# RishabhSri14/Human-Body-Reconstruction

Measured on NVIDIA B200. Metric: train_rays_per_sec, higher is better.
Workload: dtype bf16 MLP operands (f32 accumulate) / f32 encoder+compositor

## Files before the change

### human_body_reconstruction_b200/_lib.py

```python
from __future__ import annotations

import ctypes as C
import os
import subprocess
import sys
import threading

import torch

_HERE = os.path.dirname(os.path.abspath(__file__))
ROOT = os.path.dirname(_HERE)
CSRC = os.path.join(_HERE, "csrc")
SO_PATH = os.path.join(_HERE, "libhbr_b200.so")
INCLUDE = os.path.join(ROOT, "include")

NVCC_FLAGS = [
    "-gencode", "arch=compute_100a,code=sm_100a", "-O3", "-lineinfo", "-std=c++17",
    "--fmad=true",
    "-Xcompiler", "-fPIC", "-Xcompiler", "-O3", "-Xptxas", "-v",
]

HBR_MAX_LEVELS = 32
HBR_MAX_PEERS, HBR_PEER_MAX_CTAS, HBR_PEER_HANDLE_BYTES = 8, 128, 64
HBR_PEER_FLAG_BYTES = HBR_PEER_MAX_CTAS * HBR_MAX_PEERS * 4
# ... 20 lines not shown

def _deps():
    return [os.path.join(CSRC, f) for f in os.listdir(CSRC) if os.path.isfile(os.path.join(CSRC, f))] + \
        [os.path.join(INCLUDE, "hbr.h")]


def _stale() -> bool:
    if not os.path.exists(SO_PATH):
        return True
    t = os.path.getmtime(SO_PATH)
    return any(os.path.getmtime(d) > t for d in _deps())


def build(force: bool = False, verbose: bool = False) -> str:
    if not force and not _stale():
        return SO_PATH
    bdir = os.path.join(_HERE, "build")
    os.makedirs(bdir, exist_ok=True)
    import fcntl
    with open(os.path.join(bdir, ".lock"), "w") as lockf:
        fcntl.flock(lockf, fcntl.LOCK_EX)
        try:
            if not force and not _stale():
                return SO_PATH
            return _build_locked(bdir, force, verbose)
        finally:
            fcntl.flock(lockf, fcntl.LOCK_UN)


def _build_locked(bdir: str, force: bool, verbose: bool) -> str:
    nvcc = os.environ.get("NVCC", "/usr/local/cuda/bin/nvcc")
    objs, procs = [], []
    for src in sources():
        obj = os.path.join(bdir, os.path.basename(src)[:-3] + ".o")
        objs.append(obj)
        if (not force) and os.path.exists(obj) and os.path.getmtime(obj) > max(os.path.getmtime(d) for d in _deps()):
            continue
        cmd = [nvcc, *NVCC_FLAGS, *os.environ.get("HBR_EXTRA_NVCC", "").split(), "-I", INCLUDE, "-c", src, "-o", obj]
        procs.append((src, subprocess.Popen(cmd, stdout=subprocess.PIPE, stderr=subprocess.STDOUT, text=True)))
    log = []
    for src, p in procs:
        out, _ = p.communicate()
        log.append(f"== {os.path.basename(src)}\n{out}")
        if p.returncode != 0:
            raise RuntimeError(f"nvcc failed for {src}:\n{out}")
    with open(os.path.join(bdir, "ptxas.log"), "a" if not force else "w") as f:
        f.write("\n".join(log))
    if verbose:
        print("\n".join(log))
    tmp_so = os.path.join(bdir, f"libhbr_b200.{os.getpid()}.so.tmp")
    cmd = [nvcc, "-shared", "-o", tmp_so, *objs, "-lcudart"]
    r = subprocess.run(cmd, stdout=subprocess.PIPE, stderr=subprocess.STDOUT, text=True)
    if r.returncode != 0:
        raise RuntimeError(f"link failed:\n{r.stdout}")
    os.replace(tmp_so, SO_PATH)
    return SO_PATH


def build_debug(force: bool = False) -> str:
    dbg = os.path.join(CSRC, "debug")
    srcs = sorted(os.path.join(dbg, f) for f in os.listdir(dbg) if f.endswith(".cu")) + [os.path.join(CSRC, "abi.cu")]
    deps = _deps() + [os.path.join(dbg, f) for f in os.listdir(dbg)]
    if not force and os.path.exists(DEBUG_SO_PATH) and os.path.getmtime(DEBUG_SO_PATH) > max(os.path.getmtime(d) for d in deps):
        return DEBUG_SO_PATH
    nvcc = os.environ.get("NVCC", "/usr/local/cuda/bin/nvcc")
    cmd = [nvcc, *[f for f in NVCC_FLAGS if f not in ("-Xptxas", "-v")], "-I", INCLUDE, "-shared", "-o", DEBUG_SO_PATH, *srcs,
           "-lcudart"]
    r = subprocess.run(cmd, stdout=subprocess.PIPE, stderr=subprocess.STDOUT, text=True)
    if r.returncode != 0:
        raise RuntimeError(f"nvcc failed for the debug library:\n{r.stdout}")
    return DEBUG_SO_PATH


_lib = None
_debug_lib = None
_lock = threading.Lock()

_i64, _i32, _f32, _vp = C.c_int64, C.c_int, C.c_float, C.c_void_p
_geom_p, _dims_p = C.POINTER(HashGeom), C.POINTER(MlpDims)

SIGNATURES = {
    "hbr_abi_version": ([], C.c_int),
    "hbr_last_error": ([], C.c_char_p),
    "hbr_mlp_param_count": ([_dims_p], _i64),
    "hbr_mlp_act_floats": ([], _i64),
    "hbr_hash_encode_fwd": ([_vp, _i32, _i64, _vp, _geom_p, _vp, _i64, _vp], C.c_int),
    "hbr_hash_encode_bwd": ([_vp, _i32, _i64, _vp, _i64, _geom_p, _vp, _i32, _i32, _vp], C.c_int),
    "hbr_hash_encode_dx": ([_vp, _i32, _i64, _vp, _geom_p, _vp, _i64, _vp, _vp], C.c_int),
    "hbr_hash_indices": ([_vp, _i32, _i64, _geom_p, _vp, _vp, _vp], C.c_int),
    "hbr_dir_encode": ([_vp, _i32, _i64, _i32, _i32, _vp, _vp], C.c_int),
    "hbr_mlp_fwd_f32": ([_vp, _i64, _vp, _i64, _i64, _vp, _dims_p, _vp, _vp, _vp], C.c_int),
    "hbr_mlp_bwd_f32": ([_vp, _i64, _vp, _i64, _i64, _vp, _dims_p, _vp, _vp, _vp, _vp, _i64, _vp, _vp, _vp], C.c_int),
    "hbr_mlp_tc_scratch_bytes": ([_dims_p], _i64),
    "hbr_mlp_fwd_tc": ([_vp, _i32, _i64, _vp, _i64, _i64, _vp, _dims_p, _i32, _vp, _vp, _i32, _vp, _vp, _vp], C.c_int),
    "hbr_mlp_bwd_tc": ([_vp, _i32, _i64, _vp, _i64, _i64, _vp, _dims_p, _i32, _vp, _vp, _vp, _i64, _vp, _vp, _f32, _vp, _i32, _i32,
                        _vp, _vp, _vp], C.c_int),
    "hbr_occupancy_update": ([_vp, _i64, _vp, _i64, _vp, _i32, C.POINTER(C.c_float), _f32, _vp, _vp], C.c_int),
    "hbr_compact_samples": ([_vp, _vp, _vp, _i64, _i64, _i64, _vp, _i32, C.POINTER(C.c_float), _f32, _vp, _vp, _vp, _vp, _vp],
                            C.c_int),
    "hbr_hash_encode_fwd_pts": ([_vp, _i64, _vp, _vp, _geom_p, _vp, _i64, _i32, _vp], C.c_int),
    "hbr_hash_encode_bwd_pts": ([_vp, _i64, _vp, _vp, _i64, _geom_p, _vp, _i32, _i32, _vp], C.c_int),
    "hbr_mlp_tc_prepare": ([_vp, _dims_p, _i32, _vp, _vp], C.c_int),
    "hbr_mlp_tc_reduce_grads": ([_dims_p, _i64, _vp, _vp, _vp], C.c_int),
    "hbr_strat_depths": ([_vp, _vp, _f32, _f32, _i64, _vp, _vp], C.c_int),
    "hbr_mse_pair_fwd": ([_vp, _vp, _vp, _i64, _f32, _vp, _vp], C.c_int),
    "hbr_mse_pair_bwd": ([_vp, _vp, _vp, _i64, _f32, _vp, _vp, _vp, _vp], C.c_int),
    "hbr_hash_encode_fwd_rays": ([_vp, _vp, _vp, _i64, _i64, _i64, _vp, _geom_p, _vp, _i64, _i32, _vp], C.c_int),
    "hbr_field_bwd_rays_tc": ([_vp, _vp, _vp, _vp, _i64, _i64, _i64, _geom_p, _vp, _vp, _dims_p, _i32, _vp, _vp, _vp, _vp, _vp, _f32,
                               _vp, _i32, _i32, _vp], C.c_int),
    "hbr_field_fwd_rays_tc": ([_vp, _vp, _vp, _i64, _i64, _i64, _vp, _geom_p, _vp, _vp, _dims_p, _i32, _vp, _vp, _vp, _i32, _vp],
                              C.c_int),
    "hbr_hash_encode_bwd_rays": ([_vp, _vp, _vp, _i64, _i64, _i64, _vp, _i64, _geom_p, _vp, _i32, _i32, _vp], C.c_int),
    "hbr_field_fwd_tc": ([_vp, _i64, _vp, _geom_p, _vp, _i64, _vp, _dims_p, _i32, _vp, _vp, _vp, _vp], C.c_int),
    "hbr_field_bwd_tc": ([_vp, _i64, _geom_p, _vp, _i64, _vp, _dims_p, _i32, _vp, _vp, _vp, _vp, _vp, _vp, _f32, _vp, _vp],
                         C.c_int),
    "hbr_adam_step": ([_vp, _vp, _vp, _vp, _i64, C.c_double, C.c_double, C.c_double, C.c_double, C.c_double, _i32, _i64,
                       C.c_double, _vp, _vp], C.c_int),
    "hbr_adam_tick": ([_vp, _vp, _vp], C.c_int),
    "hbr_adam_step_dev": ([_vp, _vp, _vp, _vp, _i64, _vp, C.c_double, C.c_double, C.c_double, C.c_double, _i32, _vp, C.c_double,
                           _vp, _vp, _vp], C.c_int),
    "hbr_ray_gen": ([_vp, _i64, _i32, _i32, _f32, _f32, _f32, _f32, _vp, _i64, _i64, _vp, _i32, _vp, _vp, _vp, _vp, _vp, _vp],
                    C.c_int),
    "hbr_ray_bbox": ([_vp, _i64, _i32, _i32, _f32, _f32, _f32, _f32, _f32, _f32, _vp, _vp], C.c_int),
    "hbr_peer_alloc": ([C.POINTER(_vp), _i64], C.c_int),
    "hbr_peer_free": ([_vp], C.c_int),
    "hbr_peer_export": ([_vp, C.POINTER(C.c_ubyte)], C.c_int),
    "hbr_peer_import": ([C.POINTER(C.c_ubyte), C.POINTER(_vp)], C.c_int),
    "hbr_peer_release": ([_vp], C.c_int),
    "hbr_allreduce_peer": ([C.POINTER(_vp), C.POINTER(_vp), _vp, _i32, _i32, _i64, _f32, _i32, _vp, _vp], C.c_int),
    "hbr_hash_bwd_stream_tiles": ([_i64], _i64),
    "hbr_hash_encode_bwd_stream": ([_vp, _i32, _i64, _vp, _i64, _geom_p, _vp, C.POINTER(C.c_int), _i32, _vp, _vp], C.c_int),
    "hbr_hash_encode_bwd_rays_stream": ([_vp, _vp, _vp, _i64, _i64, _i64, _vp, _i64, _geom_p, _vp, C.POINTER(C.c_int), _i32, _vp,
                                         _vp], C.c_int),
    "hbr_hash_bwd_lm_ctas": ([_i64], _i64),
    "hbr_hash_encode_bwd_lm": ([_vp, _i32, _i64, _vp, _geom_p, _vp, C.POINTER(C.c_int), _i32, _vp, _vp], C.c_int),
    "hbr_hash_encode_bwd_rays_lm": ([_vp, _vp, _vp, _i64, _i64, _i64, _vp, _geom_p, _vp, C.POINTER(C.c_int), _i32, _vp, _vp],
                                    C.c_int),
    "hbr_allreduce_peer_stream": ([C.POINTER(_vp), C.POINTER(_vp), _vp, _i32, _i32, _i32, C.POINTER(_i64), C.POINTER(_i64),
                                   C.POINTER(C.c_uint), C.POINTER(C.c_int), _vp, _f32, _i32, _vp, _vp], C.c_int),
    "hbr_ray_points": ([_vp, _vp, _vp, _i64, _i64, _i64, _vp, _vp], C.c_int),
    "hbr_occupancy_mask": ([_vp, _i64, _vp, _i32, C.POINTER(C.c_float), _f32, _vp, _vp], C.c_int),
    "hbr_composite_fwd": ([_vp, _i64, _vp, _i64, _vp, _i64, _vp, _f32, _vp, _vp, _i64, _i64, _vp, _vp, _f32, _vp], C.c_int),
    "hbr_composite_bwd": ([_vp, _i64, _vp, _i64, _vp, _i64, _vp, _f32, _vp, _vp, _i64, _i64, _vp, _vp, _i64, _vp, _i64, _f32, _vp],
                          C.c_int),
    "hbr_composite_maps_fwd": ([_vp, _i64, _vp, _i64, _vp, _i64, _vp, _f32, _vp, _vp, _i64, _i64, _vp, _vp, _vp, _vp, _f32, _vp],
                               C.c_int),
    "hbr_composite_maps_bwd": ([_vp, _i64, _vp, _i64, _vp, _i64, _vp, _f32, _vp, _vp, _i64, _i64, _vp, _vp, _vp, _vp, _i64, _vp,
                                _i64, _f32, _vp], C.c_int),
    "hbr_hier_sample": ([_vp, _vp, _vp, _vp, _i64, _i64, _i32, _vp, _vp], C.c_int),
    "hbr_composite_sdf_fwd": ([_vp, _i64, _vp, _i64, _i32, _vp, _i64, _i64, _vp, _vp, _vp], C.c_int),
    "hbr_composite_sdf_bwd": ([_vp, _i64, _vp, _i64, _i32, _vp, _i64, _i64, _vp, _vp, _vp, _i64, _vp, _i64, _vp, _vp], C.c_int),
    "hbr_sdf_stencil_points": ([_vp, _i64, _f32, C.POINTER(C.c_float), C.POINTER(C.c_float), _vp, _vp], C.c_int),
    "hbr_sdf_eikonal_fwd": ([_vp, _i64, _f32, _vp, _vp, _vp], C.c_int),
    "hbr_sdf_eikonal_bwd": ([_vp, _i64, _f32, _vp, _vp, _vp], C.c_int),
    "hbr_grid_points": ([C.POINTER(C.c_double), C.POINTER(C.c_double), _i32, _i64, _i64, _vp, _vp], C.c_int),
    "hbr_grid_density": ([C.POINTER(C.c_double), C.POINTER(C.c_double), _i32, _i64, _i64, _vp, _geom_p, _vp, _dims_p,
                          _vp, _vp, _vp, _vp, _i64, _i32, _vp], C.c_int),
    "hbr_mlp_density_tf32x3": ([_vp, _i64, _vp, _dims_p, _vp, _vp], C.c_int),
    "hbr_mc_count": ([_vp, _i32, _i32, _i32, _f32, _i32, _i32, _vp, _vp], C.c_int),
    "hbr_mc_emit": ([_vp, _i32, _i32, _i32, _f32, _i32, _i32, _vp, _vp, _i64, _vp, _i64, _vp, _vp], C.c_int),
    "hbr_grid_interp": ([_vp, _i32, _i32, _i32, _i32, _vp, _i64, _vp, _vp], C.c_int),
}

DEBUG_SIGNATURES = {
    "hbr_debug_umma": ([_i32, _i32, _vp, _vp, _vp, _i32, _i32, _vp], C.c_int),
    "hbr_debug_umma_bench": ([_i32, _i32, _i32, _i32, _i32, _vp, _vp], C.c_int),
# ... 134 lines not shown
```

### human_body_reconstruction_b200/csrc/abi.cu

```cuda
#include "common.cuh"
#include <string.h>

namespace hbr {

char* err_buf() {
  static thread_local char buf[512] = {0};
  return buf;
}

int fail(int code, const char* fmt, ...) {
  va_list ap;
  va_start(ap, fmt);
  vsnprintf(err_buf(), 512, fmt, ap);
  va_end(ap);
  return code;
}

int sm_count() {
  static thread_local int cached_dev = -1, cached = 0;
  int dev = 0;
  if (cudaGetDevice(&dev) != cudaSuccess) return 148;
  if (dev != cached_dev) {
    cudaDeviceProp p;
    if (cudaGetDeviceProperties(&p, dev) != cudaSuccess) return 148;
    cached = p.multiProcessorCount;
    cached_dev = dev;
  }
  return cached;
}

}

extern "C" int hbr_abi_version(void) { return HBR_ABI_VERSION; }
extern "C" const char* hbr_last_error(void) { return hbr::err_buf(); }
```

### human_body_reconstruction_b200/csrc/common.cuh

```cuda
#pragma once
#include <cuda_runtime.h>
#include <cuda_fp16.h>
#include <cuda_bf16.h>
#include <stdint.h>
#include <stdio.h>
#include <stdarg.h>
#include "../../include/hbr.h"

namespace hbr {

char* err_buf();
int fail(int code, const char* fmt, ...);

#define HBR_REQUIRE(cond, ...)                                  \
  do {                                                          \
    if (!(cond)) return ::hbr::fail(HBR_ERR_ARG, __VA_ARGS__);  \
  } while (0)

#define HBR_CUDA(expr)                                                                         \
  do {                                                                                         \
    cudaError_t e__ = (expr);                                                                  \
    if (e__ != cudaSuccess)                                                                    \
      return ::hbr::fail(HBR_ERR_CUDA, "%s failed: %s (%s:%d)", #expr, cudaGetErrorString(e__), \
                         __FILE__, __LINE__);                                                  \
  } while (0)

#define HBR_LAUNCH_CHECK() HBR_CUDA(cudaGetLastError())

static inline cudaStream_t as_stream(void* s) { return reinterpret_cast<cudaStream_t>(s); }
static inline int64_t ceil_div(int64_t a, int64_t b) { return (a + b - 1) / b; }
static inline int64_t min64(int64_t a, int64_t b) { return a < b ? a : b; }
int sm_count();

constexpr uint32_t kPrimeY = 2654435761u;
constexpr uint32_t kPrimeZ = 805459861u;
constexpr long long kPrimeY64 = -1640531535LL;
constexpr long long kPrimeZ64 = 805459861LL;

struct HashGeom {
  float mu[3];
  float sigma;
  int L, F, E;
  uint32_t T;
  float scale[HBR_MAX_LEVELS];
};

static inline HashGeom to_device_geom(const hbr_hash_geom& g) {
  HashGeom d;
  for (int i = 0; i < 3; ++i) d.mu[i] = g.mu[i];
  d.sigma = g.sigma;
  d.L = g.L; d.F = g.F; d.E = g.E; d.T = g.T;
  for (int i = 0; i < HBR_MAX_LEVELS; ++i) d.scale[i] = i < g.L ? g.scale[i] : 0.f;
  return d;
}

static inline bool is_pow2(uint32_t v) { return v && !(v & (v - 1)); }

template <typename XT> __device__ __forceinline__ float load_coord(const XT* p);
template <> __device__ __forceinline__ float load_coord<float>(const float* p) { return __ldg(p); }
template <> __device__ __forceinline__ float load_coord<__half>(const __half* p) { return __half2float(__ldg(p)); }

__device__ __forceinline__ void cell_of(float x, float mu, float sigma, float scale, long long& cell, float& frac) {
  const float u = __fmul_rn(__fdiv_rn(__fsub_rn(x, mu), sigma), scale);
  cell = __float2ll_rz(u);
  frac = __fsub_rn(u, __ll2float_rn(cell));
}

template <bool POW2>
__device__ __forceinline__ uint32_t hash_corner(long long cx, long long cy, long long cz, uint32_t T) {
  if (POW2) {
    const uint32_t h = (uint32_t)cx ^ ((uint32_t)cy * kPrimeY) ^ ((uint32_t)cz * kPrimeZ);
    return h & (T - 1);
  } else {
    const unsigned long long a = (unsigned long long)cx;
    const unsigned long long b = (unsigned long long)cy * (unsigned long long)kPrimeY64;
    const unsigned long long c = (unsigned long long)cz * (unsigned long long)kPrimeZ64;
    long long v = (long long)(a ^ b ^ c);
    long long r = v % (long long)T;
    if (r < 0) r += (long long)T;
    return (uint32_t)r;
  }
}

__device__ __forceinline__ void corner_weights(float fx, float fy, float fz, float w[8]) {
  const float wx[2] = {__fsub_rn(1.f, fx), fx};
  const float wy[2] = {__fsub_rn(1.f, fy), fy};
  const float wz[2] = {__fsub_rn(1.f, fz), fz};
#pragma unroll
  for (int c = 0; c < 8; ++c) w[c] = __fmul_rn(__fmul_rn(wx[c & 1], wy[(c >> 1) & 1]), wz[(c >> 2) & 1]);
}

template <bool POW2>
__device__ __forceinline__ void corner_indices(long long ix, long long iy, long long iz, uint32_t T, uint32_t idx[8]) {
  if (POW2) {
    const uint32_t a[2] = {(uint32_t)ix, (uint32_t)ix + 1u};
    const uint32_t b0 = (uint32_t)iy * kPrimeY, c0 = (uint32_t)iz * kPrimeZ;
    const uint32_t b[2] = {b0, b0 + kPrimeY};
    const uint32_t c[2] = {c0, c0 + kPrimeZ};
#pragma unroll
    for (int k = 0; k < 8; ++k) idx[k] = (a[k & 1] ^ b[(k >> 1) & 1] ^ c[(k >> 2) & 1]) & (T - 1);
  } else {
#pragma unroll
    for (int k = 0; k < 8; ++k) idx[k] = hash_corner<false>(ix + (k & 1), iy + ((k >> 1) & 1), iz + ((k >> 2) & 1), T);
  }
}

constexpr unsigned kFull = 0xffffffffu;

__device__ __forceinline__ float warp_sum(float v) {
#pragma unroll
  for (int o = 16; o > 0; o >>= 1) v += __shfl_xor_sync(kFull, v, o);
  return v;
}
__device__ __forceinline__ float warp_incl_scan(float v, int lane) {
#pragma unroll
// ... 17 lines not shown
```

### human_body_reconstruction_b200/csrc/composite.cu

```cuda
#include "common.cuh"
#include <math_constants.h>

namespace hbr {

constexpr int kRaysPerCta = 8;

__global__ void ray_points_kernel(const float* __restrict__ o, const float* __restrict__ d, const float* __restrict__ t,
                                  long long t_rs, long long R, long long S, float* __restrict__ pts) {
  const long long i = (long long)blockIdx.x * blockDim.x + threadIdx.x;
  if (i >= R * S) return;
  const long long r = i / S, s = i - r * S;
  const float tt = __ldg(t + r * t_rs + s);
#pragma unroll
  for (int k = 0; k < 3; ++k) pts[i * 3 + k] = __fadd_rn(__ldg(o + r * 3 + k), __fmul_rn(__ldg(d + r * 3 + k), tt));
}

struct Mu3 { float v[3]; };
__global__ void occupancy_kernel(const float* __restrict__ pts, long long n, const uint8_t* __restrict__ grid, int G,
                                 Mu3 mu, float sigma, uint8_t* __restrict__ mask) {
  const long long i = (long long)blockIdx.x * blockDim.x + threadIdx.x;
  if (i >= n) return;
  long long q[3];
#pragma unroll
  for (int k = 0; k < 3; ++k) {
    const float u = __fmul_rn(__fdiv_rn(__fsub_rn(__ldg(pts + i * 3 + k), mu.v[k]), sigma), (float)G);
    long long c = __float2ll_rz(u);
    if (c < 0) c += G;
    c = c < 0 ? 0 : (c >= G ? G - 1 : c);
    q[k] = c;
  }
  mask[i] = grid[(q[0] * G + q[1]) * G + q[2]] ? 1 : 0;
}

template <typename XT>
__global__ void dir_encode_kernel(const XT* __restrict__ d, long long n, int dim, int nf, float* __restrict__ out) {
  const long long i = (long long)blockIdx.x * blockDim.x + threadIdx.x;
  const long long total = n * dim * nf;
  if (i >= total) return;
  const int k = (int)(i % nf);
  const long long rc = i / nf;
  float s, c;
  if (sizeof(XT) == 2) {
    const float x = __half2float(reinterpret_cast<const __half*>(d)[rc]);
    const float two_x = __half2float(__float2half_rn(2.f * x));
    const float a = __half2float(__float2half_rn(two_x * (float)k));
    s = __half2float(__float2half_rn(sinf(a)));
    c = __half2float(__float2half_rn(cosf(a)));
  } else {
    const float x = reinterpret_cast<const float*>(d)[rc];
    const float a = __fmul_rn(__fmul_rn(2.f, x), (float)k);
    s = sinf(a);
    c = cosf(a);
  }
  float* o = out + rc * (2 * nf);
  o[k] = s;
  o[nf + k] = c;
}

struct SampleIn {
  float delta, sig, p;
  bool keep;
};

__device__ __forceinline__ long long sample_row(const int32_t* __restrict__ rowmap, long long gs, int s, int S) {
  return rowmap == nullptr ? gs : (s < S ? (long long)__ldg(rowmap + gs) : -1);
}

__device__ __forceinline__ SampleIn load_sample(const float* __restrict__ tr, const float* __restrict__ sigma,
                                                long long sig_st, const uint8_t* __restrict__ mask, long long gs,
                                                int s, int S, float dnr, bool& live, long long row) {
  SampleIn q;
  live = s < S && row >= 0 && (mask == nullptr || mask[gs]);
  float delta = 0.f;
  if (s + 1 < S) delta = __fsub_rn(__ldg(tr + s + 1), __ldg(tr + s));
  q.delta = __fmul_rn(delta, dnr);
  const float raw = live ? __ldg(sigma + row * sig_st) : 0.f;
  q.keep = !(raw < -10.f);
  q.sig = q.keep ? raw : -10.f;
  q.p = s < S ? __fmul_rn(q.sig, q.delta) : 0.f;
  return q;
}

template <bool MAPS>
__global__ void __launch_bounds__(kRaysPerCta * 32)
composite_fwd_kernel(const float* __restrict__ t, long long t_rs, const float* __restrict__ rgb, long long rgb_st,
                     const float* __restrict__ sigma, long long sig_st, const float* __restrict__ dn, float dn_scalar,
                     const uint8_t* __restrict__ mask, const int32_t* __restrict__ rowmap, long long R, int S,
                     float* __restrict__ C, float* __restrict__ w_out, float ert_tau, float* __restrict__ depth,
                     float* __restrict__ opac) {
  const int lane = threadIdx.x & 31;
  const long long ray = (long long)blockIdx.x * kRaysPerCta + (threadIdx.x >> 5);
  if (ray >= R) return;
  const float* tr = t + ray * t_rs;
  const float dnr = dn ? __ldg(dn + ray) : dn_scalar;
  float carry = 0.f, c0 = 0.f, c1 = 0.f, c2 = 0.f, dsum = 0.f, asum = 0.f;
  for (int s0 = 0; s0 < S; s0 += 32) {
    const int s = s0 + lane;
    const long long gs = ray * S + s;
    bool live;
    const long long row = sample_row(rowmap, gs, s, S);
    const SampleIn q = load_sample(tr, sigma, sig_st, mask, gs, s, S, dnr, live, row);
    const float incl = carry + warp_incl_scan(q.p, lane);
    float prev = __shfl_up_sync(kFull, incl, 1);
    if (lane == 0) prev = carry;
    const float T = s == 0 ? 1.f : expf(-prev);
    const float alpha = 1.f - expf(-q.p);
    const float w = s < S ? __fmul_rn(T, alpha) : 0.f;
    if (s < S) {
      if (w_out) w_out[gs] = w;
      if (MAPS) {
        dsum += w * __ldg(tr + s);
        asum += w;
      }
      if (live) {
        const float* c = rgb + row * rgb_st;
        c0 += w * __ldg(c + 0);
        c1 += w * __ldg(c + 1);
        c2 += w * __ldg(c + 2);
      }
    }
    carry = __shfl_sync(kFull, incl, 31);
    if (carry > ert_tau) {
      if (w_out)
        for (int s2 = s0 + 32 + lane; s2 < S; s2 += 32) w_out[ray * S + s2] = 0.f;
      break;
    }
  }
  c0 = warp_sum(c0); c1 = warp_sum(c1); c2 = warp_sum(c2);
  if (lane == 0) { C[ray * 3 + 0] = c0; C[ray * 3 + 1] = c1; C[ray * 3 + 2] = c2; }
  if (MAPS) {
    dsum = warp_sum(dsum); asum = warp_sum(asum);
    if (lane == 0) {
      if (depth) depth[ray] = dsum;
      if (opac) opac[ray] = asum;
    }
  }
}

template <int NCH, bool MAPS>
__global__ void __launch_bounds__(kRaysPerCta * 32)
composite_bwd_kernel(const float* __restrict__ t, long long t_rs, const float* __restrict__ rgb, long long rgb_st,
                     const float* __restrict__ sigma, long long sig_st, const float* __restrict__ dn, float dn_scalar,
                     const uint8_t* __restrict__ mask, const int32_t* __restrict__ rowmap, long long R, int S,
                     const float* __restrict__ gC, float* __restrict__ drgb, long long drgb_st, float* __restrict__ dsig,
                     long long dsig_st, float ert_tau, const float* __restrict__ gD, const float* __restrict__ gA) {
  const int lane = threadIdx.x & 31;
  const long long ray = (long long)blockIdx.x * kRaysPerCta + (threadIdx.x >> 5);
  if (ray >= R) return;
  const float* tr = t + ray * t_rs;
  const float dnr = dn ? __ldg(dn + ray) : dn_scalar;
  float g0 = 0.f, g1 = 0.f, g2 = 0.f, gd = 0.f, ga = 0.f;
  if (!MAPS || gC) { g0 = __ldg(gC + ray * 3 + 0); g1 = __ldg(gC + ray * 3 + 1); g2 = __ldg(gC + ray * 3 + 2); }
  if (MAPS) {
    if (gD) gd = __ldg(gD + ray);
    if (gA) ga = __ldg(gA + ray);
  }
  const bool packed = drgb_st == 4 && dsig_st == 4 && dsig == drgb + 3;

  float Tk[NCH], ek[NCH], ck[NCH], dk[NCH];
  float carry = 0.f;
  bool done = false;
#pragma unroll
  for (int i = 0; i < NCH; ++i) {
    const int s = i * 32 + lane;
    Tk[i] = 0.f; ek[i] = 1.f; ck[i] = 0.f; dk[i] = 0.f;
    if (i * 32 < S && !done) {
      const long long gs = ray * S + s;
      bool live;
      const long long row = sample_row(rowmap, gs, s, S);
      const SampleIn q = load_sample(tr, sigma, sig_st, mask, gs, s, S, dnr, live, row);
      const float incl = carry + warp_incl_scan(q.p, lane);
      float prev = __shfl_up_sync(kFull, incl, 1);
      if (lane == 0) prev = carry;
      carry = __shfl_sync(kFull, incl, 31);
      if (s < S) {
        Tk[i] = s == 0 ? 1.f : expf(-prev);
        ek[i] = expf(-q.p);
        if (live) {
          const float* c = rgb + row * rgb_st;
          ck[i] = g0 * __ldg(c + 0) + g1 * __ldg(c + 1) + g2 * __ldg(c + 2);
          dk[i] = q.keep ? q.delta : 0.f;
        }
        if (MAPS) ck[i] = __fadd_rn(__fmaf_rn(gd, __ldg(tr + s), ck[i]), ga);
      }
      done = carry > ert_tau;
    }
  }
  float rcarry = 0.f;
#pragma unroll
  for (int i = NCH - 1; i >= 0; --i) {
    if (i * 32 < S) {
      const int s = i * 32 + lane;
      const long long gs = ray * S + s;
      const float w = Tk[i] * (1.f - ek[i]);
      const float wc = w * ck[i];
      const float rin = warp_rincl_scan(wc, lane);
      float after = __shfl_down_sync(kFull, rin, 1);
      if (lane == 31) after = 0.f;
      const float suffix = rcarry + after;
      rcarry += __shfl_sync(kFull, rin, 0);
      if (s < S) {
        const long long row = sample_row(rowmap, gs, s, S);
        const bool live = row >= 0 && (mask == nullptr || mask[gs]);
        const float dp = Tk[i] * ek[i] * ck[i] - suffix;
        const float ds = live ? dk[i] * dp : 0.f;
        const float r0 = live ? w * g0 : 0.f, r1 = live ? w * g1 : 0.f, r2 = live ? w * g2 : 0.f;
        if (row >= 0) {
          if (packed) {
            *reinterpret_cast<float4*>(drgb + row * 4) = make_float4(r0, r1, r2, ds);
          } else {
            float* o = drgb + row * drgb_st;
            o[0] = r0; o[1] = r1; o[2] = r2;
            dsig[row * dsig_st] = ds;
          }
        }
      }
    }
  }
}

constexpr int kHierWarps = 4;

__global__ void __launch_bounds__(kHierWarps * 32)
hier_sample_kernel(float* __restrict__ w, const float* __restrict__ t, const float* __restrict__ u,
                   const float* __restrict__ cand, long long R, int S, int P2, int clamp_in_place,
                   float* __restrict__ t_fine) {
  extern __shared__ float sm[];
  const int warp = threadIdx.x >> 5, lane = threadIdx.x & 31;
  float* cdf = sm + (size_t)warp * (S + P2);
  float* arr = cdf + S;
  const long long ray = (long long)blockIdx.x * kHierWarps + warp;
  if (ray >= R) return;
  float* wr = w + ray * S;
  float part = 0.f;
  for (int s = lane; s < S; s += 32) {
    float v = wr[s];
    if (v < 0.f) { v = 0.f; if (clamp_in_place) wr[s] = 0.f; }
    v = __fadd_rn(v, 1e-5f);
    cdf[s] = v;
    part += v;
  }
  const float total = warp_sum(part);
  __syncwarp();
  for (int s = lane; s < S; s += 32) cdf[s] = __fdiv_rn(cdf[s], total);
  __syncwarp();
  if (lane == 0) {
    float acc = 0.f;
    for (int s = 0; s < S; ++s) { acc = __fadd_rn(acc, cdf[s]); cdf[s] = acc; }
  }
  __syncwarp();
  for (int s = lane; s < P2; s += 32) {
    float v = CUDART_INF_F;
    if (s < S) {
      v = __ldg(t + s);
    } else if (s < 2 * S) {
      const float uu = __ldg(u + ray * S + (s - S));
      int lo = 0, hi = S;
      while (lo < hi) {
        const int mid = (lo + hi) >> 1;
        if (cdf[mid] <= uu) lo = mid + 1; else hi = mid;
      }
      v = __ldg(cand + min(lo, S - 1));
    }
    arr[s] = v;
  }
  __syncwarp();
  for (int k = 2; k <= P2; k <<= 1) {
    for (int j = k >> 1; j > 0; j >>= 1) {
      for (int i = lane; i < P2; i += 32) {
        const int ixj = i ^ j;
        if (ixj > i) {
          const float a = arr[i], b = arr[ixj];
          const bool asc = (i & k) == 0;
          if ((a > b) == asc) { arr[i] = b; arr[ixj] = a; }
        }
      }
      __syncwarp();
    }
  }
  for (int s = lane; s < 2 * S; s += 32) t_fine[ray * 2 * S + s] = arr[s];
}

}

using namespace hbr;

extern "C" int hbr_ray_points(const float* o, const float* d, const float* t, int64_t t_rs, int64_t R, int64_t S,
                              float* pts, void* stream) {
  HBR_REQUIRE(R >= 0 && S >= 0, "negative size");
  if (R * S == 0) return HBR_OK;
  HBR_REQUIRE(o && d && t && pts, "NULL pointer");
  HBR_REQUIRE(t_rs == 0 || t_rs >= S, "t_ray_stride %lld", (long long)t_rs);
  ray_points_kernel<<<(unsigned)ceil_div(R * S, 256), 256, 0, as_stream(stream)>>>(o, d, t, t_rs, R, S, pts);
  HBR_LAUNCH_CHECK();
  return HBR_OK;
}

extern "C" int hbr_occupancy_mask(const float* pts, int64_t n, const uint8_t* grid, int G, const float* mu3,
                                  float sigma, uint8_t* mask, void* stream) {
  if (n == 0) return HBR_OK;
  HBR_REQUIRE(pts && grid && mu3 && mask && G > 0, "bad argument");
  Mu3 mu{{mu3[0], mu3[1], mu3[2]}};
  occupancy_kernel<<<(unsigned)ceil_div(n, 256), 256, 0, as_stream(stream)>>>(pts, n, grid, G, mu, sigma, mask);
  HBR_LAUNCH_CHECK();
  return HBR_OK;
}

extern "C" int hbr_dir_encode(const void* d, int d_dtype, int64_t n, int dim, int num_freq, float* out, void* stream) {
  HBR_REQUIRE(d_dtype == HBR_F32 || d_dtype == HBR_F16, "d_dtype %d", d_dtype);
  HBR_REQUIRE(dim >= 1 && num_freq >= 1 && num_freq <= 127, "dim=%d num_freq=%d", dim, num_freq);
  if (n == 0) return HBR_OK;
  HBR_REQUIRE(d && out, "NULL pointer");
  const long long total = (long long)n * dim * num_freq;
  const unsigned grid = (unsigned)ceil_div(total, 256);
  if (d_dtype == HBR_F16) dir_encode_kernel<__half><<<grid, 256, 0, as_stream(stream)>>>((const __half*)d, n, dim, num_freq, out);
  else dir_encode_kernel<float><<<grid, 256, 0, as_stream(stream)>>>((const float*)d, n, dim, num_freq, out);
  HBR_LAUNCH_CHECK();
  return HBR_OK;
}

static int check_composite(const float* t, int64_t t_rs, const float* rgb, const float* sigma, int64_t R, int64_t S) {
  HBR_REQUIRE(R >= 0 && S >= 1 && S <= 1024, "R=%lld S=%lld (S must be 1..1024)", (long long)R, (long long)S);
  HBR_REQUIRE(t && rgb && sigma, "NULL pointer");
  HBR_REQUIRE(t_rs == 0 || t_rs >= S, "t_ray_stride %lld", (long long)t_rs);
  return HBR_OK;
}

extern "C" int hbr_composite_fwd(const float* t, int64_t t_rs, const float* rgb, int64_t rgb_st, const float* sigma,
                                 int64_t sig_st, const float* dn, float dn_scalar, const uint8_t* mask, const int32_t* rowmap,
                                 int64_t R, int64_t S, float* C, float* w, float ert_tau, void* stream) {
  if (R == 0) return HBR_OK;
  if (int rc = check_composite(t, t_rs, rgb, sigma, R, S)) return rc;
  HBR_REQUIRE(C != nullptr, "C is NULL");
  if (!(ert_tau > 0.f)) ert_tau = 3.0e38f;
  composite_fwd_kernel<false><<<(unsigned)ceil_div(R, kRaysPerCta), kRaysPerCta * 32, 0, as_stream(stream)>>>(
      t, t_rs, rgb, rgb_st, sigma, sig_st, dn, dn_scalar, mask, rowmap, R, (int)S, C, w, ert_tau, nullptr, nullptr);
  HBR_LAUNCH_CHECK();
  return HBR_OK;
}

extern "C" int hbr_composite_maps_fwd(const float* t, int64_t t_rs, const float* rgb, int64_t rgb_st, const float* sigma,
                                      int64_t sig_st, const float* dn, float dn_scalar, const uint8_t* mask,
                                      const int32_t* rowmap, int64_t R, int64_t S, float* C, float* w, float* depth,
                                      float* opacity, float ert_tau, void* stream) {
  if (R == 0) return HBR_OK;
  if (int rc = check_composite(t, t_rs, rgb, sigma, R, S)) return rc;
  HBR_REQUIRE(C != nullptr, "C is NULL");
  if (!(ert_tau > 0.f)) ert_tau = 3.0e38f;
  composite_fwd_kernel<true><<<(unsigned)ceil_div(R, kRaysPerCta), kRaysPerCta * 32, 0, as_stream(stream)>>>(
      t, t_rs, rgb, rgb_st, sigma, sig_st, dn, dn_scalar, mask, rowmap, R, (int)S, C, w, ert_tau, depth, opacity);
  HBR_LAUNCH_CHECK();
  return HBR_OK;
}

template <bool MAPS>
static int composite_bwd_launch(const float* t, int64_t t_rs, const float* rgb, int64_t rgb_st, const float* sigma,
                                int64_t sig_st, const float* dn, float dn_scalar, const uint8_t* mask, const int32_t* rowmap,
                                int64_t R, int64_t S, const float* gC, const float* gD, const float* gA, float* drgb,
                                int64_t drgb_st, float* dsig, int64_t dsig_st, float ert_tau, void* stream) {
  if (!(ert_tau > 0.f)) ert_tau = 3.0e38f;
  if (drgb_st == 4 && dsig_st == 4 && dsig == drgb + 3)
    HBR_REQUIRE((uintptr_t)drgb % 16 == 0, "packed gradient buffer must be 16-byte aligned");
  const unsigned grid = (unsigned)ceil_div(R, kRaysPerCta);
  cudaStream_t st = as_stream(stream);
#define HBR_CB(N)                                                                                                      \
  composite_bwd_kernel<N, MAPS><<<grid, kRaysPerCta * 32, 0, st>>>(t, t_rs, rgb, rgb_st, sigma, sig_st, dn, dn_scalar, \
                                                                   mask, rowmap, R, (int)S, gC, drgb, drgb_st, dsig,   \
                                                                   dsig_st, ert_tau, gD, gA)
  if (S <= 128) HBR_CB(4);
  else if (S <= 256) HBR_CB(8);
  else if (S <= 512) HBR_CB(16);
  else HBR_CB(32);
#undef HBR_CB
  HBR_LAUNCH_CHECK();
  return HBR_OK;
}

extern "C" int hbr_composite_bwd(const float* t, int64_t t_rs, const float* rgb, int64_t rgb_st, const float* sigma,
                                 int64_t sig_st, const float* dn, float dn_scalar, const uint8_t* mask, const int32_t* rowmap,
                                 int64_t R, int64_t S, const float* gC, float* drgb, int64_t drgb_st, float* dsig,
                                 int64_t dsig_st, float ert_tau, void* stream) {
  if (R == 0) return HBR_OK;
  if (int rc = check_composite(t, t_rs, rgb, sigma, R, S)) return rc;
  HBR_REQUIRE(gC && drgb && dsig, "NULL pointer");
  return composite_bwd_launch<false>(t, t_rs, rgb, rgb_st, sigma, sig_st, dn, dn_scalar, mask, rowmap, R, S, gC, nullptr,
                                     nullptr, drgb, drgb_st, dsig, dsig_st, ert_tau, stream);
}

extern "C" int hbr_composite_maps_bwd(const float* t, int64_t t_rs, const float* rgb, int64_t rgb_st, const float* sigma,
                                      int64_t sig_st, const float* dn, float dn_scalar, const uint8_t* mask,
                                      const int32_t* rowmap, int64_t R, int64_t S, const float* gC, const float* gD,
                                      const float* gA, float* drgb, int64_t drgb_st, float* dsig, int64_t dsig_st,
                                      float ert_tau, void* stream) {
  if (R == 0) return HBR_OK;
  if (int rc = check_composite(t, t_rs, rgb, sigma, R, S)) return rc;
  HBR_REQUIRE(drgb && dsig, "NULL pointer");
  return composite_bwd_launch<true>(t, t_rs, rgb, rgb_st, sigma, sig_st, dn, dn_scalar, mask, rowmap, R, S, gC, gD, gA,
                                    drgb, drgb_st, dsig, dsig_st, ert_tau, stream);
}

extern "C" int hbr_hier_sample(float* w, const float* t, const float* u, const float* cand, int64_t R, int64_t S,
                               int clamp_in_place, float* t_fine, void* stream) {
  if (R == 0) return HBR_OK;
  HBR_REQUIRE(S >= 1 && S <= 2048, "S=%lld (1..2048)", (long long)S);
  HBR_REQUIRE(w && t && u && cand && t_fine, "NULL pointer");
  int P2 = 2;
  while (P2 < 2 * S) P2 <<= 1;
  const size_t smem = (size_t)kHierWarps * (S + P2) * sizeof(float);
  HBR_CUDA(cudaFuncSetAttribute(hier_sample_kernel, cudaFuncAttributeMaxDynamicSharedMemorySize, (int)smem));
  hier_sample_kernel<<<(unsigned)ceil_div(R, kHierWarps), kHierWarps * 32, smem, as_stream(stream)>>>(
      w, t, u, cand, R, (int)S, P2, clamp_in_place, t_fine);
  HBR_LAUNCH_CHECK();
  return HBR_OK;
}
```

### human_body_reconstruction_b200/csrc/hash_grid.cu

```cuda
#include "common.cuh"

namespace hbr {

#ifndef HBR_HASH_TILE
#define HBR_HASH_TILE 128
#endif
constexpr int kTilePts = HBR_HASH_TILE;
constexpr int kHashThreads = 2 * kTilePts;

template <int F> struct FeatVec;
template <> struct FeatVec<1> { using type = float; };
template <> struct FeatVec<2> { using type = float2; };
template <> struct FeatVec<4> { using type = float4; };

template <int F>
__device__ __forceinline__ void load_feat(const float* __restrict__ base, uint32_t idx, float v[F]) {
  if (F == 1) {
    v[0] = __ldg(base + idx);
  } else if (F == 2) {
    const float2 t = __ldg(reinterpret_cast<const float2*>(base) + idx);
    v[0] = t.x; v[1] = t.y;
  } else {
    const float4 t = __ldg(reinterpret_cast<const float4*>(base) + idx);
    v[0] = t.x; v[1] = t.y; v[2] = t.z; v[3] = t.w;
  }
}

__device__ __forceinline__ void red_add_f32(float* p, float a) {
  asm volatile("red.global.add.f32 [%0], %1;" ::"l"(p), "f"(a) : "memory");
}
__device__ __forceinline__ void red_add_v2(float* p, float a, float b) {
  asm volatile("red.global.add.v2.f32 [%0], {%1, %2};" ::"l"(p), "f"(a), "f"(b) : "memory");
}
__device__ __forceinline__ void red_add_v4(float* p, float a, float b, float c, float d) {
  asm volatile("red.global.add.v4.f32 [%0], {%1, %2, %3, %4};" ::"l"(p), "f"(a), "f"(b), "f"(c), "f"(d) : "memory");
}

template <int F>
__device__ __forceinline__ void red_feat(float* base, uint32_t idx, const float v[F]) {
  if (F == 1) {
    red_add_f32(base + idx, v[0]);
  } else if (F == 2) {
    red_add_v2(base + 2 * (size_t)idx, v[0], v[1]);
  } else {
    red_add_v4(base + 4 * (size_t)idx, v[0], v[1], v[2], v[3]);
  }
}

template <typename XT>
__device__ __forceinline__ void load_point(const XT* __restrict__ x, long long gp, long long n, float p[3]) {
  if (gp < n) {
    p[0] = load_coord(x + gp * 3 + 0);
    p[1] = load_coord(x + gp * 3 + 1);
    p[2] = load_coord(x + gp * 3 + 2);
  } else {
    p[0] = p[1] = p[2] = 0.f;
  }
}

struct RaySrc {
  const float* o;
  const float* d;
  const float* t;
  long long S, t_stride;
};
struct RayPts {};
__device__ __forceinline__ void load_point(const RaySrc& rs, long long gp, long long n, float p[3]) {
  if (gp < n) {
    long long ray, smp;
    if (n <= 0xffffffffLL) {
      const unsigned q = (unsigned)gp / (unsigned)rs.S;
      ray = q;
      smp = (long long)((unsigned)gp - q * (unsigned)rs.S);
    } else {
      ray = gp / rs.S;
      smp = gp - ray * rs.S;
    }
    const float tt = __ldg(rs.t + ray * rs.t_stride + smp);
#pragma unroll
    for (int a = 0; a < 3; ++a) p[a] = __fadd_rn(__ldg(rs.o + ray * 3 + a), __fmul_rn(__ldg(rs.d + ray * 3 + a), tt));
  } else {
    p[0] = p[1] = p[2] = 0.f;
  }
}
template <typename XT> struct PointSrc { using type = const XT*; };
template <> struct PointSrc<RayPts> { using type = RaySrc; };

template <int F, bool POW2, typename XT, int PAIR = 0, int UNR = 4, typename YT = float>
__global__ void __launch_bounds__(kHashThreads)
hash_fwd_kernel(const typename PointSrc<XT>::type x, long long n, const float* __restrict__ table, YT* __restrict__ y,
                long long y_stride, const __grid_constant__ HashGeom g, int y_fmt, const unsigned long long* __restrict__ n_dev) {
  extern __shared__ float tile[];
  if (n_dev != nullptr) {
    n = min(n, (long long)__ldg(n_dev));
    if ((long long)blockIdx.x * kTilePts >= n) return;
  }
  const int C = g.L * F;
  const int pitch = C | 1;
  const int p = threadIdx.x & (kTilePts - 1);
  const int grp = threadIdx.x / kTilePts;
  const long long base = (long long)blockIdx.x * kTilePts;
  float pt[3];
  load_point(x, base + p, n, pt);

#pragma unroll UNR
  for (int l = grp; l < g.L; l += 2) {
    const float s = g.scale[l];
    long long ix, iy, iz;
    float fx, fy, fz;
    cell_of(pt[0], g.mu[0], g.sigma, s, ix, fx);
    cell_of(pt[1], g.mu[1], g.sigma, s, iy, fy);
    cell_of(pt[2], g.mu[2], g.sigma, s, iz, fz);
    uint32_t idx[8];
    corner_indices<POW2>(ix, iy, iz, g.T, idx);
    const float* lvl = table + (size_t)l * g.T * F;
    float v[8][F];
    if (F == 2 && POW2 && PAIR == 1) {
      const bool even = !(ix & 1);
#pragma unroll
      for (int c = 0; c < 8; c += 2) {
        const float4 q0 = __ldg(reinterpret_cast<const float4*>(lvl) + (idx[c] >> 1));
        float4 q1 = q0;
        if (!even) q1 = __ldg(reinterpret_cast<const float4*>(lvl) + (idx[c + 1] >> 1));
        const bool o0 = idx[c] & 1, o1 = idx[c + 1] & 1;
        v[c][0] = o0 ? q0.z : q0.x;     v[c][F - 1] = o0 ? q0.w : q0.y;
        v[c + 1][0] = o1 ? q1.z : q1.x; v[c + 1][F - 1] = o1 ? q1.w : q1.y;
      }
    } else {
#pragma unroll
      for (int c = 0; c < 8; ++c) load_feat<F>(lvl, idx[c], v[c]);
    }
    float w[8];
    corner_weights(fx, fy, fz, w);
#pragma unroll
    for (int f = 0; f < F; ++f) {
      float acc = __fmul_rn(v[0][f], w[0]);
#pragma unroll
      for (int c = 1; c < 8; ++c) acc = __fadd_rn(acc, __fmul_rn(v[c][f], w[c]));
      tile[p * pitch + l * F + f] = acc;
    }
  }
  __syncthreads();
  const int cols = C + g.E;
  const int warp = threadIdx.x >> 5, lane = threadIdx.x & 31;
  if (sizeof(YT) == 2) {
    uint32_t* y32 = reinterpret_cast<uint32_t*>(y);
    const int half = cols >> 1;
    for (int e = threadIdx.x; e < kTilePts * half; e += kHashThreads) {
      const int r = e / half, c = (e - r * half) * 2;
      const long long gp = base + r;
      if (gp >= n) break;
      const float a = c < C ? tile[r * pitch + c] : 0.f, b = c + 1 < C ? tile[r * pitch + c + 1] : 0.f;
      uint32_t v;
      if (y_fmt == HBR_F16) {
        const __half2 hh = __floats2half2_rn(a, b);
        v = *reinterpret_cast<const uint32_t*>(&hh);
      } else {
        const __nv_bfloat162 hh = __floats2bfloat162_rn(a, b);
        v = *reinterpret_cast<const uint32_t*>(&hh);
      }
      y32[(gp * y_stride + c) >> 1] = v;
    }
  } else {
    for (int r = warp; r < kTilePts; r += kHashThreads / 32) {
      const long long gp = base + r;
      if (gp >= n) break;
      for (int c = lane; c < cols; c += 32) y[gp * y_stride + c] = (YT)(c < C ? tile[r * pitch + c] : 0.f);
    }
  }
}

struct ChunkPlan {
  int nchunks;
  int bounds[HBR_MAX_LEVELS + 1];
  unsigned* done;
// ... 284 lines not shown
    corner_indices<POW2>(ix, iy, iz, g.T, idx);
    const float* lvl = table + (size_t)l * g.T * F;
    float v[8][F];
#pragma unroll
    for (int c = 0; c < 8; ++c) load_feat<F>(lvl, idx[c], v[c]);
    float gc[8];
#pragma unroll
    for (int c = 0; c < 8; ++c) {
      gc[c] = 0.f;
#pragma unroll
      for (int f = 0; f < F; ++f) gc[c] = fmaf(tile[p * pitch + l * F + f], v[c][f], gc[c]);
    }
    const float wx[2] = {1.f - fx, fx}, wy[2] = {1.f - fy, fy}, wz[2] = {1.f - fz, fz};
    float du[3] = {0.f, 0.f, 0.f};
#pragma unroll
    for (int c = 0; c < 8; ++c) {
      const int bx = c & 1, by = (c >> 1) & 1, bz = (c >> 2) & 1;
      const float sg = bx ? gc[c] : -gc[c], sy = by ? gc[c] : -gc[c], sz = bz ? gc[c] : -gc[c];
      du[0] = fmaf(sg, wy[by] * wz[bz], du[0]);
      du[1] = fmaf(sy, wx[bx] * wz[bz], du[1]);
      du[2] = fmaf(sz, wx[bx] * wy[by], du[2]);
    }
    const float k = s / g.sigma;
#pragma unroll
    for (int a = 0; a < 3; ++a) acc[a] = fmaf(k, du[a], acc[a]);
  }
  if (grp == 1) {
#pragma unroll
    for (int a = 0; a < 3; ++a) part[p * 3 + a] = acc[a];
  }
  __syncthreads();
  const long long gp = base + p;
  if (grp == 0 && gp < n) {
#pragma unroll
    for (int a = 0; a < 3; ++a) dx[gp * 3 + a] = acc[a] + part[p * 3 + a];
  }
}

static int check_geom(const hbr_hash_geom* g) {
  HBR_REQUIRE(g != nullptr, "geom is NULL");
  HBR_REQUIRE(g->L >= 1 && g->L <= HBR_MAX_LEVELS, "L=%d out of range [1,%d]", g->L, HBR_MAX_LEVELS);
  HBR_REQUIRE(g->F == 1 || g->F == 2 || g->F == 4, "F=%d unsupported (1, 2 or 4)", g->F);
  HBR_REQUIRE(g->T >= 1 && g->T <= (1u << 30), "T=%u out of range", g->T);
  HBR_REQUIRE(g->E >= 0, "E=%d negative", g->E);
  return HBR_OK;
}

template <int F, bool POW2, typename XT>
static int launch_fwd(const void* x, int64_t n, const float* table, const HashGeom& g, float* y, int64_t ys, cudaStream_t st) {
  const size_t smem = (size_t)kTilePts * ((g.L * F) | 1) * sizeof(float);
  const unsigned grid = (unsigned)ceil_div(n, kTilePts);
  auto k = hash_fwd_kernel<F, POW2, XT>;
  HBR_CUDA(cudaFuncSetAttribute(k, cudaFuncAttributeMaxDynamicSharedMemorySize, (int)smem));
  k<<<grid, kHashThreads, smem, st>>>(static_cast<const XT*>(x), n, table, y, ys, g, HBR_F32, nullptr);
  HBR_LAUNCH_CHECK();
  return HBR_OK;
}
template <int F, bool POW2, typename XT>
static int launch_bwd(const void* x, int64_t n, const float* dy, int64_t ds, const HashGeom& g, float* dt, int l0, int l1,
                      cudaStream_t st) {
  const size_t smem = (size_t)kTilePts * ((g.L * F) | 1) * sizeof(float);
  HBR_CUDA(cudaFuncSetAttribute(hash_bwd_kernel<F, POW2, XT>, cudaFuncAttributeMaxDynamicSharedMemorySize, (int)smem));
  hash_bwd_kernel<F, POW2, XT><<<(unsigned)ceil_div(n, kTilePts), kHashThreads, smem, st>>>(
      static_cast<const XT*>(x), n, dy, ds, dt, g, l0, l1, nullptr, ChunkPlan{});
  HBR_LAUNCH_CHECK();
  return HBR_OK;
}
template <int F, bool POW2, typename XT>
static int launch_dx(const void* x, int64_t n, const float* table, const float* dy, int64_t ds, const HashGeom& g, float* dx,
                     cudaStream_t st) {
  const size_t smem = (size_t)kTilePts * (((g.L * F) | 1) + 3) * sizeof(float);
  auto k = hash_dx_kernel<F, POW2, XT>;
  HBR_CUDA(cudaFuncSetAttribute(k, cudaFuncAttributeMaxDynamicSharedMemorySize, (int)smem));
  k<<<(unsigned)ceil_div(n, kTilePts), kHashThreads, smem, st>>>(static_cast<const XT*>(x), n, table, dy, ds, dx, g);
  HBR_LAUNCH_CHECK();
  return HBR_OK;
}
template <int F, bool POW2, typename YT>
static int launch_fwd_rays(const RaySrc& rs, int64_t n, const float* table, const HashGeom& g, void* y, int64_t ys, int y_fmt,
                           cudaStream_t st) {
  const size_t smem = (size_t)kTilePts * ((g.L * F) | 1) * sizeof(float);
  auto k = hash_fwd_kernel<F, POW2, RayPts, 0, 4, YT>;
  HBR_CUDA(cudaFuncSetAttribute(k, cudaFuncAttributeMaxDynamicSharedMemorySize, (int)smem));
  k<<<(unsigned)ceil_div(n, kTilePts), kHashThreads, smem, st>>>(rs, n, table, static_cast<YT*>(y), ys, g, y_fmt, nullptr);
  HBR_LAUNCH_CHECK();
  return HBR_OK;
}
template <int F, bool POW2>
static int launch_bwd_rays(const RaySrc& rs, int64_t n, const float* dy, int64_t ds, const HashGeom& g, float* dt, int l0,
                           int l1, cudaStream_t st) {
  const size_t smem = (size_t)kTilePts * ((g.L * F) | 1) * sizeof(float);
  auto k = hash_bwd_kernel<F, POW2, RayPts>;
  HBR_CUDA(cudaFuncSetAttribute(k, cudaFuncAttributeMaxDynamicSharedMemorySize, (int)smem));
  k<<<(unsigned)ceil_div(n, kTilePts), kHashThreads, smem, st>>>(rs, n, dy, ds, dt, g, l0, l1, nullptr, ChunkPlan{});

  HBR_LAUNCH_CHECK();
  return HBR_OK;
}
template <int F, bool POW2, typename YT>
static int launch_fwd_pts(const float* x, int64_t n, const unsigned long long* n_dev, const float* table, const HashGeom& g,
                          void* y, int64_t ys, int y_fmt, cudaStream_t st) {
  const size_t smem = (size_t)kTilePts * ((g.L * F) | 1) * sizeof(float);
  auto k = hash_fwd_kernel<F, POW2, float, 0, 4, YT>;
  HBR_CUDA(cudaFuncSetAttribute(k, cudaFuncAttributeMaxDynamicSharedMemorySize, (int)smem));
  k<<<(unsigned)ceil_div(n, kTilePts), kHashThreads, smem, st>>>(x, n, table, static_cast<YT*>(y), ys, g, y_fmt, n_dev);
  HBR_LAUNCH_CHECK();
  return HBR_OK;
}
template <int F, bool POW2>
static int launch_bwd_pts(const float* x, int64_t n, const unsigned long long* n_dev, const float* dy, int64_t ds,
                          const HashGeom& g, float* dt, int l0, int l1, cudaStream_t st) {
  const size_t smem = (size_t)kTilePts * ((g.L * F) | 1) * sizeof(float);
  auto k = hash_bwd_kernel<F, POW2, float>;
  HBR_CUDA(cudaFuncSetAttribute(k, cudaFuncAttributeMaxDynamicSharedMemorySize, (int)smem));
  k<<<(unsigned)ceil_div(n, kTilePts), kHashThreads, smem, st>>>(x, n, dy, ds, dt, g, l0, l1, n_dev, ChunkPlan{});
  HBR_LAUNCH_CHECK();
  return HBR_OK;
}

template <int F, bool POW2, typename XT>
static int launch_bwd_stream(const typename PointSrc<XT>::type src, int64_t n, const float* dy, int64_t ds, const HashGeom& g,
                             float* dt, ChunkPlan plan, cudaStream_t st) {
  const size_t smem = (size_t)kTilePts * ((g.L * F) | 1) * sizeof(float);
  auto k = hash_bwd_kernel<F, POW2, XT, true>;
  HBR_CUDA(cudaFuncSetAttribute(k, cudaFuncAttributeMaxDynamicSharedMemorySize, (int)smem));
  const int64_t tiles = ceil_div(n, kTilePts);
  HBR_REQUIRE(tiles * plan.nchunks < (1LL << 31), "too many CTAs: %lld tiles x %d chunks", (long long)tiles, plan.nchunks);
  plan.tiles = (unsigned)tiles;
  k<<<(unsigned)(tiles * plan.nchunks), kHashThreads, smem, st>>>(src, n, dy, ds, dt, g, 0, 0, nullptr, plan);
  HBR_LAUNCH_CHECK();
  return HBR_OK;
}
static int make_plan(const hbr_hash_geom* geom, const int* bounds, int nchunks, unsigned* done, ChunkPlan& plan) {
  HBR_REQUIRE(bounds != nullptr && done != nullptr, "NULL level_bounds / done");
  HBR_REQUIRE(nchunks >= 1 && nchunks <= geom->L, "nchunks=%d out of range [1,%d]", nchunks, geom->L);
  HBR_REQUIRE(bounds[0] == 0 && bounds[nchunks] == geom->L, "level_bounds must run from 0 to L");
  for (int c = 0; c < nchunks; ++c) HBR_REQUIRE(bounds[c] < bounds[c + 1], "level_bounds must increase");
  plan = ChunkPlan{};
  plan.nchunks = nchunks;
  for (int c = 0; c <= nchunks; ++c) plan.bounds[c] = bounds[c];
  for (int l = 0; l < geom->L; ++l) plan.order[l] = l;
  plan.done = done;
  return HBR_OK;
}

template <int F, bool POW2, typename XT>
static int launch_bwd_lm(const typename PointSrc<XT>::type src, int64_t n, const float* dy, const HashGeom& g, float* dt,
                         const ChunkPlan& plan, cudaStream_t st) {
  const int64_t ctas = ceil_div(n, kLmPts);
  HBR_REQUIRE(ctas < (1LL << 31), "too many points: %lld", (long long)n);
  hash_bwd_lm_kernel<F, POW2, XT><<<(unsigned)ctas, kLmThreads, 0, st>>>(src, n, dy, dt, g, plan);
  HBR_LAUNCH_CHECK();
  return HBR_OK;
}

#define HBR_DISPATCH_HASH(FN, ...)                                                             \
  do {                                                                                         \
    const bool p2 = is_pow2(g.T);                                                              \
    const bool h = x_dtype == HBR_F16;                                                         \
    switch (g.F) {                                                                             \
      case 1:                                                                                  \
        return p2 ? (h ? FN<1, true, __half>(__VA_ARGS__) : FN<1, true, float>(__VA_ARGS__))   \
                  : (h ? FN<1, false, __half>(__VA_ARGS__) : FN<1, false, float>(__VA_ARGS__)); \
      case 2:                                                                                  \
        return p2 ? (h ? FN<2, true, __half>(__VA_ARGS__) : FN<2, true, float>(__VA_ARGS__))   \
                  : (h ? FN<2, false, __half>(__VA_ARGS__) : FN<2, false, float>(__VA_ARGS__)); \
      default:                                                                                 \
        return p2 ? (h ? FN<4, true, __half>(__VA_ARGS__) : FN<4, true, float>(__VA_ARGS__))   \
                  : (h ? FN<4, false, __half>(__VA_ARGS__) : FN<4, false, float>(__VA_ARGS__)); \
    }                                                                                          \
  } while (0)

}

using namespace hbr;

extern "C" int hbr_hash_encode_fwd(const void* x, int x_dtype, int64_t n, const float* table,
                                   const hbr_hash_geom* geom, float* y, int64_t y_stride, void* stream) {
  if (int rc = check_geom(geom)) return rc;
  HBR_REQUIRE(x_dtype == HBR_F32 || x_dtype == HBR_F16, "x_dtype %d", x_dtype);
  HBR_REQUIRE(n >= 0 && n < (1LL << 40), "n=%lld", (long long)n);
  if (n == 0) return HBR_OK;
  HBR_REQUIRE(x && table && y, "NULL pointer");
  HBR_REQUIRE(y_stride >= geom->L * geom->F + geom->E, "y_stride %lld too small", (long long)y_stride);
  HBR_REQUIRE((uintptr_t)table % 16 == 0, "table must be 16-byte aligned");
  const HashGeom g = to_device_geom(*geom);
  HBR_DISPATCH_HASH(launch_fwd, x, n, table, g, y, y_stride, as_stream(stream));
}

// ... 286 lines not shown
```

### human_body_reconstruction_b200/csrc/mlp_tc_impl.cuh

```cuda
#ifndef HBR_OP
#error "define HBR_OP (tc::OpBf16 | tc::OpF16) and HBR_OPNS before including mlp_tc_impl.cuh"
#endif

#ifndef HBR_RING_SLOTS
#define HBR_RING_SLOTS 2
#endif

namespace hbr {
namespace HBR_OPNS {
using namespace tc;
using OP = HBR_OP;


constexpr int kTile = 128;
constexpr int kLBO128 = kTile * 16;

template <int K0P, int KCP>
struct WOfs {
  static constexpr int w0 = 0;
  static constexpr int w1 = w0 + 64 * K0P * 2;
  static constexpr int w2 = w1 + 64 * 64 * 2;
  static constexpr int w3 = w2 + 16 * 64 * 2;
  static constexpr int w4 = w3 + 64 * KCP * 2;
  static constexpr int w5 = w4 + 64 * 64 * 2;
// ... 319 lines not shown
      uint4 o;
      o.x = OP::pack_relu(p[0], p[1]); o.y = OP::pack_relu(p[2], p[3]);
      o.z = OP::pack_relu(p[4], p[5]); o.w = OP::pack_relu(p[6], p[7]);
      *reinterpret_cast<uint4*>(tile + chunk_off(r, half * 4 + cg, kTile)) = o;
    }
  }
}

__device__ __forceinline__ void masked_dz_to_tmem64(uint32_t taddr, int r, const uint8_t* tile, uint32_t taddr_a, uint4* o) {
  float v[64];
  tmem_ld<64>(taddr, v);
#pragma unroll
  for (int cg = 0; cg < 8; ++cg) {
    const uint4 h = *reinterpret_cast<const uint4*>(tile + chunk_off(r, cg, kTile));
    const float* p = v + cg * 8;
    uint4& q = o[cg];
    q.x = OP::mask_pos(OP::pack(p[0], p[1]), h.x); q.y = OP::mask_pos(OP::pack(p[2], p[3]), h.y);
    q.z = OP::mask_pos(OP::pack(p[4], p[5]), h.z); q.w = OP::mask_pos(OP::pack(p[6], p[7]), h.w);
  }
  tmem_st16(taddr_a, reinterpret_cast<const uint32_t*>(o));
  tmem_st16(taddr_a + 16, reinterpret_cast<const uint32_t*>(o) + 16);
  tmem_st_wait();
}
__device__ __forceinline__ void store_tile64(int r, uint8_t* tile, const uint4* o) {
#pragma unroll
  for (int cg = 0; cg < 8; ++cg) *reinterpret_cast<uint4*>(tile + chunk_off(r, cg, kTile)) = o[cg];
}

template <int KCP, bool PLANT_ONE>
__device__ __forceinline__ void build_cin(const float* o16, const float* __restrict__ dirs, long long dir_row, int dv,
                                          bool valid, int r, uint8_t* cin) {
#pragma unroll
  for (int cg = 0; cg < KCP / 8; ++cg) {
    float v[8];
#pragma unroll
    for (int i = 0; i < 8; ++i) {
      const int k = cg * 8 + i;
      float x = 0.f;
      if (k < kFeat) x = o16[1 + k];
      else if (k < kFeat + dv) x = valid ? __ldg(dirs + dir_row * dv + (k - kFeat)) : 0.f;
      else if (PLANT_ONE && k == kFeat + dv) x = 1.f;
      v[i] = x;
    }
    store_chunk<OP>(cin, r, cg, kTile, v);
  }
}

__device__ __forceinline__ void prefetch_l2(const void* p) { asm volatile("prefetch.global.L2 [%0];" ::"l"(p)); }
__device__ __forceinline__ void prefetch_l1(const void* p) { asm volatile("prefetch.global.L1 [%0];" ::"l"(p)); }

#define HBR_SIGNAL()          \
  do {                        \
    fence_async_smem();       \
    fence_before_sync();      \
    mbar_arrive(full);        \
  } while (0)
#define HBR_WAIT()            \
  do {                        \
    mbar_wait(done, dphase);  \
    dphase ^= 1;              \
    fence_after_sync();       \
  } while (0)

__device__ __forceinline__ long long tiles_of_slot(long long ntiles, long long slot, long long nslots) {
  return slot < ntiles ? (ntiles - slot + nslots - 1) / nslots : 0;
}

template <int K0P, int KCP>
struct Scratch {
  static constexpr int off_bias = WOfs<K0P, KCP>::total;
  static constexpr int off_ones16 = off_bias + BOfs::total;
  static constexpr int off_bias_f32 = off_ones16 + kTile * 16 * 2;
  static constexpr int off_grad = (off_bias_f32 + 6 * 64 * 4 + 255) & ~255;
  static constexpr int kMaxRows = 256;
  static constexpr int kRowFloats = 18432;
  static constexpr long long total = (long long)off_grad + (long long)kMaxRows * kRowFloats * 4;
};

constexpr int kPrepCtas = 11;
template <int K0P, int KCP>
__global__ void __launch_bounds__(256) mlp_prep_kernel(const float* __restrict__ params, int in0, int dv, uint8_t* img) {
  using SC = Scratch<K0P, KCP>;
  const MlpLayout m = make_layout(in0, dv);
  if (blockIdx.x < kPrepCtas - 2) {
    constexpr int kChunks = WOfs<K0P, KCP>::total / 16;
    const int c = blockIdx.x * 256 + threadIdx.x;
    if (c < kChunks) stage_weights_bf16<K0P, KCP>(params, m, img, nullptr, nullptr, nullptr, false, c, 1 << 30);
  } else if (blockIdx.x == kPrepCtas - 2) {
    stage_weights_bf16<K0P, KCP>(params, m, img, img + SC::off_bias, img + SC::off_ones16, nullptr, true);
  } else {
    stage_weights_bf16<K0P, KCP>(params, m, img, nullptr, nullptr, reinterpret_cast<float*>(img + SC::off_bias_f32), true);
  }
}

__device__ __forceinline__ void cp_async16(void* dst, const void* src, bool valid) {
  asm volatile("cp.async.cg.shared.global [%0], [%1], 16, %2;\n" ::"r"(smem_u32(dst)), "l"(src), "r"(valid ? 16 : 0) : "memory");
}
__device__ __forceinline__ void cp_async_commit() { asm volatile("cp.async.commit_group;\n" ::: "memory"); }
__device__ __forceinline__ void cp_async_wait_all() { asm volatile("cp.async.wait_group 0;\n" ::: "memory"); }

__device__ __forceinline__ void copy_image_async(uint8_t* dst, const uint8_t* __restrict__ src, int bytes) {
  for (int e = threadIdx.x; e < bytes / 16; e += blockDim.x) cp_async16(dst + e * 16, src + e * 16, true);
  cp_async_commit();
}

constexpr int kReduceSlices = 8;
__global__ void __launch_bounds__(256) mlp_grad_reduce_kernel(const float* __restrict__ rows, int nrows, int row_floats,
                                                               int total, float* __restrict__ dparams) {
  const int e = blockIdx.x * blockDim.x + threadIdx.x;
  if (e >= total) return;
  const int per = (nrows + kReduceSlices - 1) / kReduceSlices;
  const int r0 = blockIdx.y * per, r1 = min(nrows, r0 + per);
  float acc = 0.f;
#pragma unroll 4
  for (int r = r0; r < r1; ++r) acc += __ldg(rows + (size_t)r * row_floats + e);
  if (r1 > r0) atomicAdd(dparams + e, acc);
}


__device__ __forceinline__ void encode_row(const EncArgs& e, const HashGeom& g, long long gp, long long n, int r, uint8_t* x0) {
  float pt[3] = {0.f, 0.f, 0.f};
  if (gp < n) {
    pt[0] = __ldg(e.x + gp * 3 + 0); pt[1] = __ldg(e.x + gp * 3 + 1); pt[2] = __ldg(e.x + gp * 3 + 2);
  }
  uint32_t packed[16];
#pragma unroll 2
  for (int l = 0; l < 16; ++l) {
    const float s = g.scale[l];
    long long ix, iy, iz;
    float fx, fy, fz;
    cell_of(pt[0], g.mu[0], g.sigma, s, ix, fx);
    cell_of(pt[1], g.mu[1], g.sigma, s, iy, fy);
    cell_of(pt[2], g.mu[2], g.sigma, s, iz, fz);
    uint32_t idx[8];
    corner_indices<true>(ix, iy, iz, g.T, idx);
    const float* lvl = e.table + (size_t)l * g.T * 2;
    float v[8][2];
    if (!(ix & 1)) {
#pragma unroll
      for (int c = 0; c < 8; c += 2) {
        const float4 q = __ldg(reinterpret_cast<const float4*>(lvl) + (idx[c] >> 1));
        const bool odd = idx[c] & 1;
        v[c][0] = odd ? q.z : q.x;     v[c][1] = odd ? q.w : q.y;
        v[c + 1][0] = odd ? q.x : q.z; v[c + 1][1] = odd ? q.y : q.w;
      }
    } else {
#pragma unroll
      for (int c = 0; c < 8; ++c) {
        const float2 q = __ldg(reinterpret_cast<const float2*>(lvl) + idx[c]);
        v[c][0] = q.x; v[c][1] = q.y;
      }
    }
    float w[8];
    corner_weights(fx, fy, fz, w);
    float a0 = __fmul_rn(v[0][0], w[0]), a1 = __fmul_rn(v[0][1], w[0]);
#pragma unroll
    for (int c = 1; c < 8; ++c) {
      a0 = __fadd_rn(a0, __fmul_rn(v[c][0], w[c]));
      a1 = __fadd_rn(a1, __fmul_rn(v[c][1], w[c]));
    }
    packed[l] = OP::pack(a0, a1);
  }
#pragma unroll
  for (int cg = 0; cg < 4; ++cg) {
    const uint4 q = make_uint4(packed[4 * cg], packed[4 * cg + 1], packed[4 * cg + 2], packed[4 * cg + 3]);
    *reinterpret_cast<uint4*>(x0 + chunk_off(r, cg, kTile)) = q;
    if (gp < n) reinterpret_cast<uint4*>(e.feat16 + gp * 32)[cg] = q;
  }
}

__device__ __forceinline__ void load_feat16_row(const EncArgs& e, long long gp, long long n, int r, uint8_t* x0) {
#pragma unroll
  for (int cg = 0; cg < 4; ++cg) {
    const uint4 q = gp < n ? __ldg(reinterpret_cast<const uint4*>(e.feat16 + gp * 32) + cg) : make_uint4(0, 0, 0, 0);
    *reinterpret_cast<uint4*>(x0 + chunk_off(r, cg, kTile)) = q;
  }
}

__device__ __forceinline__ void scatter_row(const EncArgs& e, const HashGeom& g, const float pt[3], bool valid, int lane,
                                            const float* df) {
#pragma unroll 1
  for (int l = 0; l < 16; ++l) {
    const float s = g.scale[l];
    long long ix, iy, iz;
    float fx, fy, fz;
    cell_of(pt[0], g.mu[0], g.sigma, s, ix, fx);
    cell_of(pt[1], g.mu[1], g.sigma, s, iy, fy);
    cell_of(pt[2], g.mu[2], g.sigma, s, iz, fz);
    float w[8];
    corner_weights(fx, fy, fz, w);
    float g0 = 0.f, g1 = 0.f;
// ... 98 lines not shown
    cell_of_norm(un[1], s, iy, fy);
    cell_of_norm(un[2], s, iz, fz);
    uint32_t idx[8];
    corner_indices<true>(ix, iy, iz, g.T, idx);
    const float2* lvl = reinterpret_cast<const float2*>(e.table) + (size_t)l * g.T;
#pragma unroll
    for (int c = 0; c < 8; ++c) v[q][c] = __ldg(lvl + idx[c]);
    fr[q][0] = fx; fr[q][1] = fy; fr[q][2] = fz;
  }
  uint32_t packed[NLV];
#pragma unroll
  for (int q = 0; q < NLV; ++q) {
    float w[8];
    corner_weights(fr[q][0], fr[q][1], fr[q][2], w);
    float a0 = __fmul_rn(v[q][0].x, w[0]), a1 = __fmul_rn(v[q][0].y, w[0]);
#pragma unroll
    for (int c = 1; c < 8; ++c) {
      a0 = __fadd_rn(a0, __fmul_rn(v[q][c].x, w[c]));
      a1 = __fadd_rn(a1, __fmul_rn(v[q][c].y, w[c]));
    }
    packed[q] = OP::pack(a0, a1);
  }
  if constexpr (NLV == 4) {
    const uint4 out4 = make_uint4(packed[0], packed[1], packed[2], packed[3]);
    *reinterpret_cast<uint4*>(x0 + chunk_off(r, lg, kTile)) = out4;
    if (gp < n) reinterpret_cast<uint4*>(e.feat16 + gp * 32)[lg] = out4;
  } else {
    const uint2 out2 = make_uint2(packed[0], packed[1]);
    *reinterpret_cast<uint2*>(x0 + chunk_off(r, lg >> 1, kTile) + (lg & 1) * 8) = out2;
    if (gp < n) reinterpret_cast<uint2*>(e.feat16 + gp * 32)[lg] = out2;
  }
}


template <int K0P, int NT = kTile>
__device__ __forceinline__ void stage_features_async(const float* __restrict__ feat, long long tile0, long long n, int gt,
                                                     uint8_t* stage) {
  constexpr int kQ = K0P / 4;
  const float4* src = reinterpret_cast<const float4*>(feat + tile0 * K0P);
#pragma unroll
  for (int it = 0; it < kTile * kQ / NT; ++it) {
    const int idx = it * NT + gt;
    const bool ok = tile0 + idx / kQ < n;
    cp_async16(stage + idx * 16, ok ? (const void*)(src + idx) : (const void*)feat, ok);
  }
  cp_async_commit();
}
template <int K0P, int NT = kTile>
__device__ __forceinline__ void convert_staged_features(const uint8_t* stage, int gt, uint8_t* x0) {
  constexpr int kQ = K0P / 4;
#pragma unroll
  for (int it = 0; it < kTile * kQ / NT; ++it) {
    const int idx = it * NT + gt, row = idx / kQ, c4 = idx % kQ;
    const float4 q = *reinterpret_cast<const float4*>(stage + idx * 16);
    uint2 o;
    o.x = OP::pack(q.x, q.y);
    o.y = OP::pack(q.z, q.w);
    *reinterpret_cast<uint2*>(x0 + chunk_off(row, c4 >> 1, kTile) + (c4 & 1) * 8) = o;
  }
}

template <int K0P, int NPART>
__device__ __forceinline__ void copy_feat16_async(const uint16_t* __restrict__ feat16, long long tile0, long long n, int r, int part,
                                                  uint8_t* dst_tile) {
  constexpr int kPer = K0P / 8 / NPART;
  const long long gp = tile0 + r;
  const bool ok = gp < n;
  const uint16_t* src = feat16 + (ok ? gp : 0) * K0P;
#pragma unroll
  for (int c = 0; c < kPer; ++c) {
    const int cg = part * kPer + c;
    cp_async16(dst_tile + chunk_off(r, cg, kTile), src + cg * 8, ok);
  }
  cp_async_commit();
}

template <int K0P, int KCP, int G, bool TRACE = false, bool ENC = false, int GATH = 0>
__global__ void __launch_bounds__(G * kTile + GATH * 32, 1)
mlp_fwd_tc_kernel(const float* __restrict__ feat, long long feat_stride, const float* __restrict__ dirs, long long dir_group,
                  long long n_arg, const float* __restrict__ params, int in0, int dv, float* __restrict__ out,
                  const uint8_t* __restrict__ image, long long* __restrict__ trace, const EncArgs enc,
                  const __grid_constant__ HashGeom geom, int feat16, const unsigned long long* __restrict__ n_dev,
                  const int32_t* __restrict__ dir_rows) {
  const long long n = n_dev != nullptr ? min(n_arg, (long long)__ldg(n_dev)) : n_arg;
  using SM = FwdSmem<K0P, KCP, G>;
  using WO = WOfs<K0P, KCP>;
  constexpr int kGrpCols = 96;
  constexpr int kCols = G * kGrpCols <= 128 ? 128 : (G * kGrpCols <= 256 ? 256 : 512);
  static_assert(G * kGrpCols <= 512, "TMEM budget exceeded");
  extern __shared__ __align__(128) uint8_t sm[];
  const MlpLayout m = make_layout(in0, dv);
  uint8_t* wsm = sm;
  uint64_t* bars = reinterpret_cast<uint64_t*>(sm + SM::off_bar);
  uint32_t* tslot = reinterpret_cast<uint32_t*>(bars + 2 * G);
  const int warp = __shfl_sync(kFull, (int)(threadIdx.x >> 5), 0), lane = threadIdx.x & 31;

  uint64_t* xfull = reinterpret_cast<uint64_t*>(sm + SM::off_xbar);
  uint64_t* xempty = xfull + 2 * G;
  constexpr int kXBuf = kTile * K0P * 2;
  static_assert(GATH == 0 || (K0P == 32 && !ENC && 2 * kXBuf <= SM::buf_bytes), "gather variant: 32 features, two buffers");
  if (warp == 0) tmem_alloc<kCols>(tslot);
  if (threadIdx.x == 32) {
    for (int g = 0; g < G; ++g) mbar_init(bars + G + g, 1);
    if (GATH > 0)
      for (int q = 0; q < 2 * G; ++q) {
        mbar_init(xfull + q, GATH * 32);
        mbar_init(xempty + q, 1);
      }
    fence_mbar_init();
  }
  if (GATH == 0) {
    if (image != nullptr) {
      copy_image_async(sm, image, SM::off_buf);
      cp_async_wait_all();
    } else {
      stage_weights_bf16<K0P, KCP>(params, m, wsm, sm + SM::off_bias, sm + SM::off_ones16);
    }
    fence_async_smem();
  }
  fence_before_sync();
  __syncthreads();
  fence_after_sync();
  const uint32_t tbase = *tslot;
  const long long ntiles = (n + kTile - 1) / kTile;
  const long long nslots = (long long)gridDim.x * G;

  constexpr int kNlv = GATH > 8 ? 2 : 4;
  constexpr int kUnits = 64 / kNlv;
  if (GATH > 0 && warp >= 4 * G) {
    if (GATH > 8) asm volatile("setmaxnreg.dec.sync.aligned.u32 %0;\n" ::"n"(56));
    const int gw = warp - 4 * G;
    uint32_t epar = 0;
#pragma unroll 1
    for (long long k = 0;; ++k) {
      bool any = false;
#pragma unroll 1
      for (int g = 0; g < G; ++g) {
        const long long tile = (long long)g * gridDim.x + blockIdx.x + k * nslots;
        if (tile >= ntiles) continue;
        any = true;
        const int slot = (int)(k & 1), q = 2 * g + slot;
        if (k >= 2) {
          mbar_wait(xempty + q, (epar >> q) & 1u);
          epar ^= 1u << q;
        }
        uint8_t* x0 = sm + SM::off_buf + g * SM::buf_bytes + slot * kXBuf;
#pragma unroll 1
        for (int u = gw; u < kUnits; u += GATH) gather_unit<kNlv>(enc, geom, n, tile, u & 3, u >> 2, lane, x0);
        fence_async_smem();
        mbar_arrive(xfull + q);
      }
      if (!any) break;
    }
  } else {
    if (GATH > 8) asm volatile("setmaxnreg.inc.sync.aligned.u32 %0;\n" ::"n"(128));
    if (GATH > 0) {
      if (image != nullptr) {
        for (int e = threadIdx.x; e < SM::off_buf / 16; e += G * kTile) cp_async16(sm + e * 16, image + e * 16, true);
        cp_async_commit();
        cp_async_wait_all();
      } else {
        stage_weights_bf16<K0P, KCP>(params, m, wsm, sm + SM::off_bias, sm + SM::off_ones16, nullptr, false, threadIdx.x,
                                     G * kTile);
      }
      fence_async_smem();
      asm volatile("bar.sync 7, %0;" ::"n"(G * kTile) : "memory");
    }
    const int g = warp >> 2;
    const int r = threadIdx.x & (kTile - 1);
    const bool issuer = (warp & 3) == 0;
    uint8_t* buf = sm + SM::off_buf + g * SM::buf_bytes;
    uint64_t* done = bars + G + g;
    const uint32_t tgrp = tbase + g * kGrpCols;
    const uint32_t taddr = tgrp + ((uint32_t)((warp & 3) * 32) << 16);
    const uint32_t taddr_a = taddr + 64;
    const uint32_t wa = a4_of(wsm), ba = a4_of(sm + SM::off_bias), o16a = a4_of(sm + SM::off_ones16), xa = a4_of(buf);
    uint32_t dphase = 0;
    const bool vec_ok = in0 == K0P && feat_stride == K0P && ((uintptr_t)feat & 15) == 0;
    int tgi = 0, tmi = 0;
    (void)tgi; (void)tmi;
    int tgk = 0;
    uint32_t xpar = 0;
    (void)tgk; (void)xpar;
    uint8_t* stage = sm + SM::off_stage + g * SM::stage_bytes;
    const bool f16in = !ENC && GATH == 0 && feat16 != 0;
    const uint16_t* featq = reinterpret_cast<const uint16_t*>(feat);
    const bool staged = !ENC && GATH == 0 && !f16in && vec_ok && SM::stage_bytes > 0;
    if (staged && (long long)g * gridDim.x + blockIdx.x < ntiles)
      stage_features_async<K0P>(feat, ((long long)g * gridDim.x + blockIdx.x) * kTile, n, r, stage);
    if (f16in && (long long)g * gridDim.x + blockIdx.x < ntiles)
      copy_feat16_async<K0P, 1>(featq, ((long long)g * gridDim.x + blockIdx.x) * kTile, n, r, 0, buf);
#define TR()                                                                                  \
  do {                                                                                        \
// ... 189 lines not shown
                                             int nthreads) {
  using TM = BwdTmem<K0P, KCP, WORK>;
  constexpr bool kCinOne = TM::kCinOne;
  if (dparams == nullptr) return;
  float* row = grad_rows != nullptr ? grad_rows + (size_t)blockIdx.x * Scratch<K0P, KCP>::kRowFloats : nullptr;
  if (!has_tiles) {
    if (row != nullptr)
      for (int e = threadIdx.x; e < m.total; e += nthreads) row[e] = 0.f;
    return;
  }
  if (warp >= 4 * ngroups) return;
  const int wq = warp & 3, unit = warp >> 2, units = ngroups;
  const uint32_t trow = tbase + ((uint32_t)(wq * 32) << 16);
  auto put = [&](int idx, float v) {
    if (row != nullptr) row[idx] = v * ginv;
    else atomicAdd(dparams + idx, v * ginv);
  };
  const int q = wq * 16 + lane;
#pragma unroll 1
  for (int t = 0; t < 4; ++t) {
    if ((t % units) != unit) continue;
    const int i = t < 2 ? t : t + 1;
    const int gcol = t == 0 ? TM::g0 : t == 1 ? TM::g1 : t == 2 ? TM::g3 : TM::g4;
    const int ncol = t == 0 ? TM::n0 : t == 1 ? TM::n1 : t == 2 ? TM::n3 : TM::n4;
    const int Ki = m.K[i], Ji = m.J[i], Wi = m.W[i], bi = m.b[i];
    const int bias_col = (i == 3 && kCinOne) ? Ki : (i == 0 ? K0P : (i == 3 ? KCP : 64));
    const bool mine = lane < 16 && q < Ji;
    const bool vec = row != nullptr && (Ki & 3) == 0 && (Wi & 3) == 0;
    const int base = Wi + q * Ki;
#pragma unroll 1
    for (int c = 0; c < ncol; c += 8) {
      float v[8];
      tmem_ld8_wait(trow + gcol + c, v);
      if (mine) {
        if (vec) {
          if (c < Ki) *reinterpret_cast<float4*>(row + base + c) = make_float4(v[0] * ginv, v[1] * ginv, v[2] * ginv, v[3] * ginv);
          if (c + 4 < Ki) *reinterpret_cast<float4*>(row + base + c + 4) = make_float4(v[4] * ginv, v[5] * ginv, v[6] * ginv, v[7] * ginv);
        } else {
#pragma unroll
          for (int j = 0; j < 8; ++j)
            if (c + j < Ki) put(base + c + j, v[j]);
        }
        if ((bias_col & ~7) == c) {
          float bv = v[0];
#pragma unroll
          for (int j = 1; j < 8; ++j)
            if ((bias_col & 7) == j) bv = v[j];
          put(bi + q, bv);
        }
      }
    }
  }
  const int r = wq * 32 + lane;
#pragma unroll 1
  for (int t = 0; t < 2; ++t) {
    if (((t + 2) % units) != unit) continue;
    const int i = t == 0 ? 2 : 5;
    const int Ji = m.J[i], Wi = m.W[i], bi = m.b[i];
    float gacc[16];
    tmem_ld<16>(trow + (t == 0 ? TM::g2 : TM::g5), gacc);
#pragma unroll
    for (int j = 0; j < 16; ++j) {
      if (j < Ji) {
        if (r < 64) put(Wi + j * 64 + r, gacc[j]);
        else if (r == 64) put(bi + j, gacc[j]);
      }
    }
  }
}

constexpr int kGroupRegs = 168;
__host__ __device__ constexpr int scat_regs(int G) { return G == 2 ? 88 : 112; }


template <int K0P, int KCP, int G, bool TRACE = false, bool ENC = false, int SCAT = 0>
__global__ void __launch_bounds__(G * kTile + SCAT * 32 + 32, 1)
mlp_bwd_tc_kernel(const float* __restrict__ feat, long long feat_stride, const float* __restrict__ dirs, long long dir_group,
                  long long n_arg, const float* __restrict__ params, int in0, int dv, const float* __restrict__ out,
                  const float* __restrict__ dout, float* __restrict__ dfeat, long long dfeat_stride,
                  float* __restrict__ ddirs, float* __restrict__ dparams, const uint8_t* __restrict__ image,
                  float* __restrict__ grad_rows, long long* __restrict__ trace, const EncArgs enc,
                  const __grid_constant__ HashGeom geom, float gscale, int feat16, const unsigned long long* __restrict__ n_dev,
                  const int32_t* __restrict__ dir_rows) {
  const long long n = n_dev != nullptr ? min(n_arg, (long long)__ldg(n_dev)) : n_arg;
  const float ginv = 1.f / gscale;
  using SM = BwdSmem<K0P, KCP, G>;
  using WO = WOfs<K0P, KCP>;
  constexpr int kGrpCols = 96;
  using TM = BwdTmem<K0P, KCP, 2 * kGrpCols>;
  constexpr bool kCinOne = TM::kCinOne;
  static_assert(G >= 1 && G <= 2, "two work accumulators");
  extern __shared__ __align__(128) uint8_t sm[];
  const MlpLayout m = make_layout(in0, dv);
  uint8_t* wsm = sm;
  float* bias = reinterpret_cast<float*>(sm + SM::off_bias);
  uint64_t* bars = reinterpret_cast<uint64_t*>(sm + SM::off_bar);
  constexpr int kSlots = SM::ring_slots;
  uint32_t* tslot = reinterpret_cast<uint32_t*>(bars + 4 * G + 2 * kSlots);
  uint64_t* dfull = bars + 4 * G;
  uint64_t* dempty = bars + 4 * G + kSlots;
  const int warp = __shfl_sync(kFull, (int)(threadIdx.x >> 5), 0), lane = threadIdx.x & 31;
  constexpr int kIssuerWarp = 4 * G + SCAT;
  if (TRACE && blockIdx.x == 0 && threadIdx.x == 0) trace[2000] = clock64();

  if (warp == 0) tmem_alloc<512>(tslot);
  if (threadIdx.x == 32) {
    for (int g = 0; g < G; ++g) {
      mbar_init(bars + G + g, 1);
      mbar_init(bars + 2 * G + g, 1);
      mbar_init(bars + 3 * G + g, 1);
    }
    for (int q = 0; q < kSlots; ++q) {
      mbar_init(dfull + q, kTile);
      mbar_init(dempty + q, SCAT > 0 ? SCAT * 32 : 1);
    }
    fence_mbar_init();
  }
  if (image != nullptr) {
    copy_image_async(wsm, image, WO::total);
    copy_image_async(sm + SM::off_bias, image + Scratch<K0P, KCP>::off_bias_f32, 6 * 64 * 4);
  } else {
    stage_weights_bf16<K0P, KCP>(params, m, wsm, nullptr, nullptr, bias);
  }
  {
    for (int e = threadIdx.x; e < G * SM::grp_bytes / 16; e += blockDim.x)
      reinterpret_cast<uint4*>(sm + SM::off_grp)[e] = make_uint4(0, 0, 0, 0);
    __syncthreads();
    const uint32_t one2 = OP::pack(1.f, 1.f);
    const uint4 ones4 = make_uint4(one2, one2, one2, one2);
    for (int e = threadIdx.x; e < kTile; e += blockDim.x) {
      for (int g = 0; g < G; ++g) {
        uint8_t* gb = sm + SM::off_grp + g * SM::grp_bytes;
        reinterpret_cast<uint4*>(gb + SM::h2 + 8 * kCg)[e] = ones4;
        reinterpret_cast<uint4*>(gb + SM::c2 + 8 * kCg)[e] = ones4;
        reinterpret_cast<uint4*>(gb + SM::x0 + kTile * K0P * 2)[e] = ones4;
        reinterpret_cast<uint4*>(gb + SM::h1 + 8 * kCg)[e] = ones4;
        reinterpret_cast<uint4*>(gb + SM::c1 + 8 * kCg)[e] = ones4;
      }
    }
  }
  cp_async_wait_all();
  fence_async_smem();
  fence_before_sync();
  __syncthreads();
  fence_after_sync();
  const uint32_t tbase = *tslot;
  if (TRACE && blockIdx.x == 0 && threadIdx.x == 0) trace[2001] = clock64();
  const long long ntiles = (n + kTile - 1) / kTile;
  const long long nslots = (long long)gridDim.x * G;
  long long nt[G];
  long long cta_tiles = 0;
#pragma unroll
  for (int g = 0; g < G; ++g) {
    nt[g] = tiles_of_slot(ntiles, (long long)g * gridDim.x + blockIdx.x, nslots);
    cta_tiles += nt[g];
  }
  const long long kmax = nt[0];

  auto wgrad_issuer = [&]() {
    const uint32_t tb0 = __shfl_sync(kFull, tbase, 0);
    const uint32_t sm0 = a4_of(sm);
    uint32_t par[G];
#pragma unroll
    for (int g = 0; g < G; ++g) par[g] = 0;
    bool first = true;
#define HBR_WGRAD_STAGE(BODY)                                              \
  _Pragma("unroll") for (int g = 0; g < G; ++g) {                          \
    if (k < nt[g]) {                                                       \
      mbar_wait(bars + 3 * G + g, par[g]);                                 \
      par[g] ^= 1;                                                         \
      fence_after_sync();                                                  \
      if (elect_one()) {                                                   \
        uint32_t sb = sm0, tb = tb0;                                       \
        asm volatile("" : "+r"(sb), "+r"(tb));                             \
        const uint32_t base = sb + (SM::off_grp + g * SM::grp_bytes) / 16; \
        const uint32_t x0a = base + SM::x0 / 16, h1a = base + SM::h1 / 16, h2a = base + SM::h2 / 16, \
                       cina = base + SM::cin / 16, c1a = base + SM::c1 / 16, c2a = base + SM::c2 / 16, \
                       dzsa = base + SM::dzs / 16;                         \
        (void)x0a; (void)h1a; (void)h2a; (void)cina; (void)c1a; (void)c2a; (void)dzsa; \
        const bool acc = !(first && g == 0);                               \
        BODY;                                                              \
        commit(bars + 2 * G + g);                                          \
      }                                                                    \
      __syncwarp();                                                        \
    }                                                                      \
  }
    for (long long k = 0; k < kmax; ++k) {
      HBR_WGRAD_STAGE(issue_wgrad(tb + TM::g5, c2a, dzsa, 16, acc, 128));
      HBR_WGRAD_STAGE(issue_wgrad(tb + TM::g4, c2a, c1a, TM::n4, acc));
      HBR_WGRAD_STAGE(issue_wgrad(tb + TM::g3, c1a, cina, TM::n3, acc));
      HBR_WGRAD_STAGE(issue_wgrad(tb + TM::g2, h2a, dzsa, 16, acc, 128));
      HBR_WGRAD_STAGE(issue_wgrad(tb + TM::g1, h2a, h1a, TM::n1, acc));
      HBR_WGRAD_STAGE(issue_wgrad(tb + TM::g0, h1a, x0a, TM::n0, acc));
      first = false;
    }
  };
  if (SCAT > 0 && warp >= 4 * G) {
    asm volatile("setmaxnreg.dec.sync.aligned.u32 %0;\n" ::"n"(scat_regs(G)));
    if (warp == kIssuerWarp) {
      wgrad_issuer();
    } else {
      const int sw = warp - 4 * G;
      constexpr int kUnits = 64;
      uint32_t fpar = 0;
      int pbuf = 0;
#pragma unroll 1
      for (long long kg = 0; kg < kmax * G; ++kg) {
        const long long k = kg / G;
        const int g = (int)(kg - k * G);
        if (k >= (g == 0 ? nt[0] : nt[G - 1])) continue;
        const long long tile = (long long)g * gridDim.x + blockIdx.x + k * nslots;
        float* pos = reinterpret_cast<float*>(sm + SM::off_pos) + pbuf * (kTile * 3);
        pbuf ^= 1;
        if (sw < 4) {
          const long long gp = tile * kTile + sw * 32 + lane;
          float x3[3] = {0.f, 0.f, 0.f};
          if (gp < n) {
            long long ray, smp;
            if (gp < (1LL << 31) && enc.S < (1LL << 31)) {
              const unsigned q = (unsigned)gp / (unsigned)enc.S;
              ray = q; smp = (long long)((unsigned)gp - q * (unsigned)enc.S);
            } else {
// ... 330 lines not shown
      HBR_BSTAGE_BWD(issue_dgrad_ts(tgrp, tgrp_a, wa + WO::w0 / 16, 64, K0P),
                     { HBR_WAIT_B(); store_tile64(r, h1, dzt); });
      if (SCAT > 0) {
        float df[K0P];
        tmem_ld<K0P>(taddr, df);
        const int slot = G == 2 ? g : (tgi % kSlots);
        if (G == 1 && tgi >= kSlots) {
          mbar_wait(dempty + slot, (ephase >> slot) & 1u);
          ephase ^= 1u << slot;
        }
        float2* stg = reinterpret_cast<float2*>(G == 2 ? h2 : sm + SM::off_ring + slot * SM::ring_slot);
#pragma unroll
        for (int l = 0; l < K0P / 2; ++l) stg[l * kTile + r] = make_float2(df[2 * l] * ginv, df[2 * l + 1] * ginv);
        mbar_arrive(dfull + slot);
      } else if (ENC) {
        float df[K0P];
        tmem_ld<K0P>(taddr, df);
#pragma unroll
        for (int k = 0; k < K0P; ++k) df[k] *= ginv;
        scatter_row(enc, geom, pt, valid, lane, df);
      } else if (dfeat != nullptr) {
        float df[K0P];
        tmem_ld<K0P>(taddr, df);
#pragma unroll
        for (int k = 0; k < K0P; ++k) df[k] *= ginv;
        if (dlm) {
          float2* stg = reinterpret_cast<float2*>(h2);
#pragma unroll
          for (int l = 0; l < K0P / 2; ++l) stg[l * kTile + r] = make_float2(df[2 * l], df[2 * l + 1]);
          asm volatile("bar.sync %0, 128;" ::"r"(1 + g) : "memory");
          const float4* s4 = reinterpret_cast<const float4*>(h2);
#pragma unroll
          for (int it = 0; it < K0P / 4; ++it) {
            const int idx = it * kTile + r, l = idx >> 6, j = idx & 63;
            if (tile * kTile + 2 * j < n)
              reinterpret_cast<float4*>(dfeat + ((size_t)l * n + tile * kTile) * 2)[j] = s4[idx];
          }
        } else if (dvec_ok) {
          constexpr int kQ = K0P / 4;
          float4* stg = reinterpret_cast<float4*>(h2);
#pragma unroll
          for (int c = 0; c < kQ; ++c)
            stg[r * kQ + (c ^ (r & 7))] = make_float4(df[4 * c], df[4 * c + 1], df[4 * c + 2], df[4 * c + 3]);
          asm volatile("bar.sync %0, 128;" ::"r"(1 + g) : "memory");
          float4* dst = reinterpret_cast<float4*>(dfeat + tile * kTile * K0P);
#pragma unroll
          for (int it = 0; it < kQ; ++it) {
            const int idx = it * kTile + r, row = idx / kQ, c = idx % kQ;
            if (tile * kTile + row < n) dst[idx] = stg[row * kQ + (c ^ (row & 7))];
          }
        } else if (valid) {
#pragma unroll
          for (int k = 0; k < K0P; ++k)
            if (k < in0) dfeat[gp * dfeat_stride + k] = df[k];
        }
      }
      HBR_STAMP(0);
      HBR_WAIT_B();
      HBR_STAMP(0);
    }
    if (TRACE && blockIdx.x == 0 && threadIdx.x == 0) trace[2004] = clock64();
  }
  fence_before_sync();
  __syncthreads();
  fence_after_sync();
  if (TRACE && blockIdx.x == 0 && threadIdx.x == 0) trace[2002] = clock64();

  if (warp < 4 * G) flush_gradients<K0P, KCP, 2 * kGrpCols>(tbase, warp, lane, G, m, cta_tiles > 0, dparams, grad_rows, ginv, 4 * G * 32);
  fence_before_sync();
  __syncthreads();
  if (TRACE && blockIdx.x == 0 && threadIdx.x == 0) trace[2003] = clock64();
  if (warp == 0) tmem_dealloc<512>(tbase);
}

static inline bool narrow_shape(const hbr_mlp_dims* d) { return d->in0 <= 32 && d->d_view + kFeat <= 40; }

template <int K0P, int KCP, int G, bool ENC>
static int launch_fwd_tc(const float* feat, int64_t feat_stride, const float* dirs, int64_t dir_group, int64_t n,
                         const float* params, int in0, int dv, float* out, uint8_t* scratch, const EncArgs& enc,
                         const HashGeom& geom, int feat16, int image_ready, const unsigned long long* n_dev, const int32_t* dir_rows,
                         cudaStream_t st) {
  constexpr int smem = FwdSmem<K0P, KCP, G>::total;
  const int grid = (int)min64(ceil_div(ceil_div(n, kTile), G), sm_count());
  if (scratch != nullptr && !image_ready) mlp_prep_kernel<K0P, KCP><<<kPrepCtas, 256, 0, st>>>(params, in0, dv, scratch);
  auto kern = mlp_fwd_tc_kernel<K0P, KCP, G, false, ENC>;
  HBR_CUDA(cudaFuncSetAttribute(kern, cudaFuncAttributeMaxDynamicSharedMemorySize, smem));
  kern<<<grid, G * kTile, smem, st>>>(feat, feat_stride, dirs, dir_group, n, params, in0, dv, out, scratch, nullptr, enc,
                                             geom, feat16, n_dev, dir_rows);
  HBR_LAUNCH_CHECK();
  return HBR_OK;
}

template <int GATH>
static int launch_fwd_gather_tc(const float* dirs, int64_t dir_group, int64_t n, const float* params, int dv, float* out,
                                const uint8_t* image, const EncArgs& enc, const HashGeom& geom, cudaStream_t st) {
  constexpr int G = 2;
  constexpr int smem = FwdSmem<32, 48, G>::total;
  const int grid = (int)min64(ceil_div(ceil_div(n, kTile), G), sm_count());
  auto kern = mlp_fwd_tc_kernel<32, 48, G, false, false, GATH>;
  HBR_CUDA(cudaFuncSetAttribute(kern, cudaFuncAttributeMaxDynamicSharedMemorySize, smem));
  kern<<<grid, G * kTile + GATH * 32, smem, st>>>(nullptr, 32, dirs, dir_group, n, params, 32, dv, out, image, nullptr, enc, geom,
                                                  1, nullptr, nullptr);
  HBR_LAUNCH_CHECK();
  return HBR_OK;
}

template <int K0P, int KCP, int G, bool ENC, int SCAT = 0>
static int launch_bwd_tc(const float* feat, int64_t feat_stride, const float* dirs, int64_t dir_group, int64_t n,
                         const float* params, int in0, int dv, const float* out, const float* dout, float* dfeat,
                         int64_t dfeat_stride, float* ddirs, float* dparams, uint8_t* scratch, const EncArgs& enc,
                         const HashGeom& geom, float gscale, int feat16, int image_ready, int defer_reduce,
                         const unsigned long long* n_dev, const int32_t* dir_rows, cudaStream_t st) {
  using SC = Scratch<K0P, KCP>;
  constexpr int smem = BwdSmem<K0P, KCP, G>::total;
  const int grid = (int)min64(ceil_div(ceil_div(n, kTile), G), sm_count());
  const bool rows = scratch != nullptr && dparams != nullptr && grid <= SC::kMaxRows;
  if (scratch != nullptr && !image_ready) mlp_prep_kernel<K0P, KCP><<<kPrepCtas, 256, 0, st>>>(params, in0, dv, scratch);
  auto kern = mlp_bwd_tc_kernel<K0P, KCP, G, false, ENC, SCAT>;
  HBR_CUDA(cudaFuncSetAttribute(kern, cudaFuncAttributeMaxDynamicSharedMemorySize, smem));
  if constexpr (SCAT > 0) {
    static_assert((G == 2 && SCAT == 7) || (G == 1 && SCAT == 11), "register budget: 16 warps, 4 per sub-partition");
    constexpr int kScatRegs = scat_regs(G);
    static int regs = 0;
    if (regs == 0) {
      cudaFuncAttributes fa;
      HBR_CUDA(cudaFuncGetAttributes(&fa, kern));
      regs = fa.numRegs;
    }
    HBR_REQUIRE(regs >= kScatRegs && regs <= kGroupRegs && 4 * regs <= 512 && G * kGroupRegs + (4 - G) * kScatRegs <= 4 * regs,
                "fused backward kernel compiled with %d registers per thread: the setmaxnreg budget does not hold", regs);
  }
  kern<<<grid, G * kTile + SCAT * 32 + 32, smem, st>>>(feat, feat_stride, dirs, dir_group, n, params, in0, dv, out, dout, dfeat,
                                           dfeat_stride, ddirs, dparams, scratch,
                                           rows ? reinterpret_cast<float*>(scratch + SC::off_grad) : nullptr, nullptr, enc, geom, gscale, feat16, n_dev, dir_rows);
  if (rows && !defer_reduce) {
    const int total = make_layout(in0, dv).total;
    mlp_grad_reduce_kernel<<<dim3((total + 255) / 256, kReduceSlices), 256, 0, st>>>(
        reinterpret_cast<const float*>(scratch + SC::off_grad), grid, SC::kRowFloats, total, dparams);
  }
  HBR_LAUNCH_CHECK();
  return HBR_OK;
}

template <int K0P, int KCP, int G>
static int reduce_grads_tc(int64_t n, int in0, int dv, uint8_t* scratch, float* dparams, cudaStream_t st) {
  using SC = Scratch<K0P, KCP>;
  const int grid = (int)min64(ceil_div(ceil_div(n, kTile), G), sm_count());
  HBR_REQUIRE(grid <= SC::kMaxRows, "grid %d exceeds the gradient rows", grid);
  const int total = make_layout(in0, dv).total;
  mlp_grad_reduce_kernel<<<dim3((total + 255) / 256, kReduceSlices), 256, 0, st>>>(
      reinterpret_cast<const float*>(scratch + SC::off_grad), grid, SC::kRowFloats, total, dparams);
  HBR_LAUNCH_CHECK();
  return HBR_OK;
}
template <int K0P, int KCP>
static int prepare_tc(const float* params, int in0, int dv, uint8_t* scratch, cudaStream_t st) {
  mlp_prep_kernel<K0P, KCP><<<kPrepCtas, 256, 0, st>>>(params, in0, dv, scratch);
  HBR_LAUNCH_CHECK();
  return HBR_OK;
}


}
}
```

### human_body_reconstruction_b200/csrc/occupancy.cu

```cuda
#include "common.cuh"

namespace hbr {

struct Mu3o { float v[3]; };

__device__ __forceinline__ long long grid_cell(const float p[3], const Mu3o& mu, float sigma, int G) {
  long long q[3];
#pragma unroll
  for (int k = 0; k < 3; ++k) {
    const float u = __fmul_rn(__fdiv_rn(__fsub_rn(p[k], mu.v[k]), sigma), (float)G);
    long long c = __float2ll_rz(u);
    if (c < 0) c += G;
    c = c < 0 ? 0 : (c >= G ? G - 1 : c);
    q[k] = c;
  }
  return (q[0] * G + q[1]) * G + q[2];
}

__global__ void occupancy_update_kernel(const float* __restrict__ pts, long long n, const float* __restrict__ alpha,
                                        long long alpha_stride, uint8_t* __restrict__ grid, int G, Mu3o mu, float sigma,
                                        unsigned* __restrict__ any) {
  const long long i = (long long)blockIdx.x * blockDim.x + threadIdx.x;
  bool hit = false;
  if (i < n && __ldg(alpha + i * alpha_stride) > 0.f) {
    const float p[3] = {__ldg(pts + i * 3), __ldg(pts + i * 3 + 1), __ldg(pts + i * 3 + 2)};
    grid[grid_cell(p, mu, sigma, G)] = 1;
    hit = true;
  }
  if (__any_sync(kFull, hit) && (threadIdx.x & 31) == 0) atomicOr(any, 1u);
}
__global__ void occupancy_finish_kernel(uint8_t* __restrict__ grid, long long cells, unsigned* __restrict__ any, unsigned* __restrict__ done) {
  const bool none = *reinterpret_cast<volatile unsigned*>(any) == 0u;
  if (none)
    for (long long i = (long long)blockIdx.x * blockDim.x + threadIdx.x; i < cells; i += (long long)gridDim.x * blockDim.x) grid[i] = 1;
  __syncthreads();
  if (threadIdx.x == 0 && atomicAdd(done, 1u) == gridDim.x - 1) { *any = 0u; *done = 0u; }
}

constexpr int kCompactWarps = 8;
constexpr int kMaxChunks = 32;

__global__ void __launch_bounds__(kCompactWarps * 32)
compact_samples_kernel(const float* __restrict__ o, const float* __restrict__ d, const float* __restrict__ t, long long t_rs,
                       long long R, int S, const uint8_t* __restrict__ grid, int G, Mu3o mu, float sigma,
                       float* __restrict__ pts_c, int32_t* __restrict__ ray_c, int32_t* __restrict__ rowmap,
                       unsigned long long* __restrict__ count) {
  const int lane = threadIdx.x & 31;
  const long long ray = (long long)blockIdx.x * kCompactWarps + (threadIdx.x >> 5);
  if (ray >= R) return;
  const float ox = __ldg(o + ray * 3), oy = __ldg(o + ray * 3 + 1), oz = __ldg(o + ray * 3 + 2);
  const float dx = __ldg(d + ray * 3), dy = __ldg(d + ray * 3 + 1), dz = __ldg(d + ray * 3 + 2);
  const float* tr = t + ray * t_rs;
  unsigned bits[kMaxChunks];
  int total = 0;
#pragma unroll
  for (int c = 0; c < kMaxChunks; ++c) {
    bits[c] = 0u;
    if (c * 32 < S) {
      const int s = c * 32 + lane;
      bool live = false;
      if (s < S) {
        const float tt = __ldg(tr + s);
        const float p[3] = {__fadd_rn(ox, __fmul_rn(dx, tt)), __fadd_rn(oy, __fmul_rn(dy, tt)), __fadd_rn(oz, __fmul_rn(dz, tt))};
        live = grid[grid_cell(p, mu, sigma, G)] != 0;
      }
      bits[c] = __ballot_sync(kFull, live);
      total += __popc(bits[c]);
    }
  }
  unsigned long long base = 0;
  if (lane == 0 && total > 0) base = atomicAdd(count, (unsigned long long)total);
  base = __shfl_sync(kFull, base, 0);
  int before = 0;
#pragma unroll
  for (int c = 0; c < kMaxChunks; ++c) {
    if (c * 32 < S) {
      const int s = c * 32 + lane;
      if (s < S) {
        const bool live = (bits[c] >> lane) & 1u;
        long long row = -1;
        if (live) {
          row = (long long)base + before + __popc(bits[c] & ((1u << lane) - 1u));
          const float tt = __ldg(tr + s);
          pts_c[row * 3 + 0] = __fadd_rn(ox, __fmul_rn(dx, tt));
          pts_c[row * 3 + 1] = __fadd_rn(oy, __fmul_rn(dy, tt));
          pts_c[row * 3 + 2] = __fadd_rn(oz, __fmul_rn(dz, tt));
          ray_c[row] = (int32_t)ray;
        }
        rowmap[ray * S + s] = (int32_t)row;
      }
      before += __popc(bits[c]);
    }
  }
}

}

using namespace hbr;

extern "C" int hbr_occupancy_update(const float* pts, int64_t n, const float* alpha, int64_t alpha_stride, uint8_t* grid, int G,
                                    const float* mu3, float sigma, unsigned int* flags2, void* stream) {
  HBR_REQUIRE(n >= 0 && G > 0 && grid && mu3 && flags2, "bad argument");
  HBR_REQUIRE(n == 0 || (pts && alpha), "NULL pointer");
  Mu3o mu{{mu3[0], mu3[1], mu3[2]}};
  cudaStream_t st = as_stream(stream);
  if (n > 0) {
    occupancy_update_kernel<<<(unsigned)ceil_div(n, 256), 256, 0, st>>>(pts, n, alpha, alpha_stride, grid, G, mu, sigma, flags2);
    HBR_LAUNCH_CHECK();
  }
  const long long cells = (long long)G * G * G;
  occupancy_finish_kernel<<<(unsigned)min64(ceil_div(cells, 256 * 16), 1024), 256, 0, st>>>(grid, cells, flags2, flags2 + 1);
  HBR_LAUNCH_CHECK();
  return HBR_OK;
}

extern "C" int hbr_compact_samples(const float* rays_o, const float* rays_d, const float* t, int64_t t_ray_stride, int64_t R,
                                   int64_t S, const uint8_t* grid, int G, const float* mu3, float sigma, float* pts_c,
                                   int32_t* ray_c, int32_t* rowmap, unsigned long long* count, void* stream) {
  HBR_REQUIRE(R >= 0 && S >= 1 && S <= 32 * kMaxChunks, "R=%lld S=%lld (S must be 1..1024)", (long long)R, (long long)S);
  HBR_REQUIRE(R * S < (1LL << 31), "R*S=%lld does not fit the 32-bit row map", (long long)(R * S));
  HBR_REQUIRE(t_ray_stride == 0 || t_ray_stride >= S, "t_ray_stride %lld", (long long)t_ray_stride);
  if (R == 0) return HBR_OK;
  HBR_REQUIRE(rays_o && rays_d && t && grid && G > 0 && mu3 && pts_c && ray_c && rowmap && count, "NULL pointer");
  Mu3o mu{{mu3[0], mu3[1], mu3[2]}};
  compact_samples_kernel<<<(unsigned)ceil_div(R, kCompactWarps), kCompactWarps * 32, 0, as_stream(stream)>>>(
      rays_o, rays_d, t, t_ray_stride, R, (int)S, grid, G, mu, sigma, pts_c, ray_c, rowmap, count);
  HBR_LAUNCH_CHECK();
  return HBR_OK;
}
```

### human_body_reconstruction_b200/csrc/step_glue.cu

```cuda
#include "common.cuh"

namespace hbr {

__global__ void strat_depths_kernel(const float* __restrict__ lin, const float* __restrict__ u, float span, float count,
                                    long long S, float* __restrict__ t) {
  const long long i = (long long)blockIdx.x * blockDim.x + threadIdx.x;
  if (i < S) t[i] = __fadd_rn(__ldg(lin + i), __fdiv_rn(__fmul_rn(__ldg(u + i), span), count));
}

__global__ void __launch_bounds__(256)
mse_pair_fwd_kernel(const float* __restrict__ a, const float* __restrict__ b, const float* __restrict__ gt, long long n,
                    double inv_n, float* __restrict__ loss) {
  float facc = 0.f;
  for (long long i = (long long)blockIdx.x * blockDim.x + threadIdx.x; i < n; i += (long long)gridDim.x * blockDim.x) {
    const float g = __ldg(gt + i);
    const float da = __ldg(a + i) - g;
    facc = fmaf(da, da, facc);
    if (b != nullptr) {
      const float db = __ldg(b + i) - g;
      facc = fmaf(db, db, facc);
    }
  }
  double acc = (double)facc;
#pragma unroll
  for (int o = 16; o > 0; o >>= 1) acc += __shfl_xor_sync(kFull, acc, o);
  __shared__ double part[8];
  const int warp = threadIdx.x >> 5, lane = threadIdx.x & 31;
  if (lane == 0) part[warp] = acc;
  __syncthreads();
  if (threadIdx.x == 0) {
    double s = 0.0;
    for (int w = 0; w < 8; ++w) s += part[w];
    atomicAdd(loss, (float)(s * inv_n));
  }
}
__global__ void mse_pair_bwd_kernel(const float* __restrict__ a, const float* __restrict__ b, const float* __restrict__ gt,
                                    long long n, float two_over_n, const float* __restrict__ gout, float* __restrict__ da,
                                    float* __restrict__ db) {
  const long long i = (long long)blockIdx.x * blockDim.x + threadIdx.x;
  if (i >= n) return;
  const float s = __ldg(gout) * two_over_n, g = __ldg(gt + i);
  da[i] = s * (__ldg(a + i) - g);
  if (b != nullptr) db[i] = s * (__ldg(b + i) - g);
}

}

using namespace hbr;

extern "C" int hbr_strat_depths(const float* lin, const float* u, float span, float count, int64_t S, float* t, void* stream) {
  HBR_REQUIRE(S >= 0 && count != 0.f, "S=%lld count=%g", (long long)S, (double)count);
  if (S == 0) return HBR_OK;
  HBR_REQUIRE(lin && u && t, "NULL pointer");
  strat_depths_kernel<<<(unsigned)ceil_div(S, 256), 256, 0, as_stream(stream)>>>(lin, u, span, count, S, t);
  HBR_LAUNCH_CHECK();
  return HBR_OK;
}

extern "C" int hbr_mse_pair_fwd(const float* a, const float* b, const float* gt, int64_t n, float scale, float* loss,
                                void* stream) {
  HBR_REQUIRE(n >= 1 && a && gt && loss, "bad argument");
  const int grid = (int)min64(ceil_div(n, 256 * 4), (long long)sm_count() * 4);
  mse_pair_fwd_kernel<<<grid, 256, 0, as_stream(stream)>>>(a, b, gt, n, (double)scale / (double)n, loss);
  HBR_LAUNCH_CHECK();
  return HBR_OK;
}

extern "C" int hbr_mse_pair_bwd(const float* a, const float* b, const float* gt, int64_t n, float scale, const float* gout,
                                float* da, float* db, void* stream) {
  HBR_REQUIRE(n >= 1 && a && gt && gout && da && (b == nullptr || db != nullptr), "bad argument");
  mse_pair_bwd_kernel<<<(unsigned)ceil_div(n, 256), 256, 0, as_stream(stream)>>>(a, b, gt, n, 2.f * scale / (float)n, gout, da, db);
  HBR_LAUNCH_CHECK();
  return HBR_OK;
}
```

### human_body_reconstruction_b200/graph.py

```python
from __future__ import annotations

from typing import Callable, Iterable, Optional

import torch


def default_loss(Cr, Cf, gt):
    from . import ops
    if Cr.is_cuda and Cr.dtype == torch.float32 and gt.dtype == torch.float32 and Cr.shape == gt.shape:
        return ops.mse_pair(Cr, None, gt, 2.0) if Cf is Cr else ops.mse_pair(Cr, Cf, gt)
    if Cf is Cr:
        return 2.0 * torch.nn.functional.mse_loss(Cr, gt)
    return torch.nn.functional.mse_loss(Cr, gt) + torch.nn.functional.mse_loss(Cf, gt)


class GraphedStep:
    def __init__(self, renderer, model, params: Iterable[torch.nn.Parameter], n_rays: int, num_samples: int,
                 hierarchical: bool, device, loss_fn: Callable = default_loss, autocast: bool = True, warmup: int = 3,
                 source=None, autocast_dtype: torch.dtype = torch.bfloat16, optimizers: Iterable = ()):
        self.renderer, self.model = renderer, model
        self.source = source
        self.params = list(params)
        self.num_samples, self.hierarchical = int(num_samples), bool(hierarchical)
        self.loss_fn, self.autocast, self.autocast_dtype = loss_fn, autocast, autocast_dtype
        self.optimizers = list(optimizers)
        for o in self.optimizers:
            if not getattr(o, "capturable", False):
                raise ValueError("optimisers captured in the step's graph must be capturable (optim.FusedAdam(capturable=True))")
        dev = torch.device(device)
        self.n_rays = int(n_rays)
        self.packed = torch.zeros(10 * n_rays, device=dev)
        R = n_rays
        self.rays_o = self.packed[0:3 * R].view(R, 3)
        self.rays_d = self.packed[3 * R:6 * R].view(R, 3)
        self.dir_norm = self.packed[6 * R:7 * R].view(R, 1)
        self.gt = self.packed[7 * R:10 * R].view(R, 3)
        self.rays_d[:, 2] = 1.0
        self.dir_norm.fill_(1.0)
        self.loss: Optional[torch.Tensor] = None
        self.graph: Optional[torch.cuda.CUDAGraph] = None
        self._warmup = warmup

    def _step(self):
        rays_o, rays_d, dir_norm, gt = self.rays_o, self.rays_d, self.dir_norm, self.gt
        if self.source is not None:
            rays_o, rays_d, dir_norm, gt = self.source.sample(self.n_rays)
        with torch.autocast("cuda", dtype=self.autocast_dtype, enabled=self.autocast):
            Cr, Cf, _ = self.renderer.vol_render(self.model, rays_d, rays_o, num_samples=self.num_samples,
                                                 update_mask=False, dir_norm=dir_norm, hierarchical=self.hierarchical)
            loss = self.loss_fn(Cr, Cf, gt)
        loss.backward()
        for o in self.optimizers:
            o.step()
        return loss

    @staticmethod
    def pack_batch(rays_o, rays_d, dir_norm, gt, pin: bool = False) -> torch.Tensor:
        flat = torch.cat([rays_o.reshape(-1), rays_d.reshape(-1), dir_norm.reshape(-1), gt.reshape(-1)]).float().contiguous()
        return flat.pin_memory() if pin and not flat.is_cuda else flat

    def load(self, rays_o, rays_d=None, dir_norm=None, gt=None, non_blocking: bool = True):
        if rays_d is None:
            self.packed.copy_(rays_o, non_blocking=non_blocking)
            return
        self.rays_o.copy_(rays_o, non_blocking=non_blocking)
        self.rays_d.copy_(rays_d, non_blocking=non_blocking)
        self.dir_norm.copy_(dir_norm.reshape(-1, 1), non_blocking=non_blocking)
        self.gt.copy_(gt, non_blocking=non_blocking)

    def capture(self):
        quiet = getattr(torch.autograd.graph, "set_warn_on_accumulate_grad_stream_mismatch", None)
        if quiet is not None:
            quiet(False)
        s = torch.cuda.Stream()
        s.wait_stream(torch.cuda.current_stream())
        with torch.cuda.stream(s):
            for _ in range(self._warmup):
                for p in self.params:
                    p.grad = None
                self._step()
        torch.cuda.current_stream().wait_stream(s)
        torch.cuda.synchronize()
        for p in self.params:
            p.grad = None
        self.graph = torch.cuda.CUDAGraph()
        with torch.cuda.graph(self.graph):
            self.loss = self._step()
        return self

    def __call__(self, rays_o=None, rays_d=None, dir_norm=None, gt=None) -> torch.Tensor:
        if self.graph is None:
            self.capture()
        if rays_o is not None:
            self.load(rays_o, rays_d, dir_norm, gt)
        self.graph.replay()
        return self.loss
```

### human_body_reconstruction_b200/ops.py

```python
from __future__ import annotations

import ctypes as C
from typing import Optional, Sequence

import torch

from . import _lib
HAS_TC = True

from ._lib import HBR_BF16, HBR_F16, HBR_F32, HashGeom, MlpDims, check, lib, ptr, require_cuda, stream


def make_geom(mu, sigma, scales: Sequence[float], L: int, F: int, T: int, E: int = 0) -> HashGeom:
    g = HashGeom()
    for i in range(3):
        g.mu[i] = float(mu[i])
    g.sigma = float(sigma)
    g.L, g.F, g.E, g.T = int(L), int(F), int(E), int(T)
    for i in range(L):
        g.scale[i] = float(scales[i])
    return g


def _xdtype(x: torch.Tensor) -> int:
# ... 441 lines not shown

class CompositeSdfPacked(torch.autograd.Function):

    @staticmethod
    def forward(ctx, out4, b, R, S, from_density=True):
        require_cuda(out4, b)
        out4 = _f32c(out4)
        b32 = b.detach().reshape(1).float().contiguous()
        Cc, w = _composite_sdf_fwd(out4, 4, out4[:, 3:], 4, int(bool(from_density)), b32, R, S)
        ctx.save_for_backward(out4, b32)
        ctx.meta = (R, S, int(bool(from_density)), b.shape, b.dtype)
        ctx.set_materialize_grads(False)
        return Cc, w

    @staticmethod
    def backward(ctx, gC, gw):
        out4, b32 = ctx.saved_tensors
        R, S, from_density, b_shape, b_dtype = ctx.meta
        d4, db = _composite_sdf_bwd(out4, 4, out4[:, 3:], 4, from_density, b32, R, S, gC, gw)
        return d4, db.reshape(b_shape).to(b_dtype), None, None, None


def sdf_stencil_points(x: torch.Tensor, eps: float, lo, hi) -> torch.Tensor:
    require_cuda(x)
    x = _f32c(x)
    n = x.shape[0]
    pts = torch.empty((6, n, 3), device=x.device, dtype=torch.float32)
    lo3, hi3 = (C.c_float * 3)(*lo), (C.c_float * 3)(*hi)
    check(lib().hbr_sdf_stencil_points(ptr(x), n, float(eps), lo3, hi3, ptr(pts), stream()))
    return pts


class SdfEikonal(torch.autograd.Function):

    @staticmethod
    def forward(ctx, dens6, eps):
        require_cuda(dens6)
        dens6 = _f32c(dens6)
        n = dens6.shape[1]
        norm = torch.empty((n,), device=dens6.device, dtype=torch.float32)
        grads = torch.empty((n, 3), device=dens6.device, dtype=torch.float32)
        check(lib().hbr_sdf_eikonal_fwd(ptr(dens6), n, float(eps), ptr(norm), ptr(grads), stream()))
        ctx.save_for_backward(dens6)
        ctx.eps = float(eps)
        ctx.mark_non_differentiable(grads)
        return norm, grads

    @staticmethod
    def backward(ctx, gnorm, _ggrads):
        (dens6,) = ctx.saved_tensors
        n = dens6.shape[1]
        dd = torch.empty_like(dens6)
        check(lib().hbr_sdf_eikonal_bwd(ptr(dens6), n, ctx.eps, ptr(_f32c(gnorm)), ptr(dd), stream()))
        return dd, None


def hier_sample(w: torch.Tensor, t: torch.Tensor, u: torch.Tensor, cand: torch.Tensor, clamp_in_place=False) -> torch.Tensor:
    require_cuda(w, t, u, cand)
    R, S = w.shape
    assert w.dtype == torch.float32 and w.is_contiguous()
    t, u, cand = _f32c(t), _f32c(u), _f32c(cand)
    tf = torch.empty((R, 2 * S), device=w.device, dtype=torch.float32)
    check(lib().hbr_hier_sample(ptr(w), ptr(t), ptr(u), ptr(cand), R, S, 1 if clamp_in_place else 0, ptr(tf), stream()))
    return tf


def strat_depths(lin: torch.Tensor, u: torch.Tensor, span: float, count: float) -> torch.Tensor:
    require_cuda(lin, u)
    lin, u = _f32c(lin), _f32c(u)
    t = torch.empty_like(lin)
    check(lib().hbr_strat_depths(ptr(lin), ptr(u), float(span), float(count), lin.numel(), ptr(t), stream()))
    return t


class MsePair(torch.autograd.Function):

    @staticmethod
    def forward(ctx, a, b, gt, scale=1.0):
        require_cuda(a, b, gt)
        a, gt = _f32c(a), _f32c(gt)
        b = _f32c(b) if b is not None else None
        if a.shape != gt.shape or (b is not None and b.shape != gt.shape):
            raise ValueError("MsePair: shapes differ")
        loss = torch.zeros((), device=a.device, dtype=torch.float32)
        check(lib().hbr_mse_pair_fwd(ptr(a), ptr(b), ptr(gt), a.numel(), float(scale), ptr(loss), stream()))
        ctx.save_for_backward(a, b, gt)
        ctx.scale = float(scale)
        return loss

    @staticmethod
    def backward(ctx, gout):
        a, b, gt = ctx.saved_tensors
        da = torch.empty_like(a)
        db = torch.empty_like(b) if b is not None else None
        gout = _f32c(gout)
        check(lib().hbr_mse_pair_bwd(ptr(a), ptr(b), ptr(gt), a.numel(), ctx.scale, ptr(gout), ptr(da), ptr(db), stream()))
        return da, db, None, None


def mse_pair(a: torch.Tensor, b: Optional[torch.Tensor], gt: torch.Tensor, scale: float = 1.0) -> torch.Tensor:
    return MsePair.apply(a, b, gt, scale)


def mlp_act_rows() -> int:
    return int(lib().hbr_mlp_act_floats())


def mlp_fwd_f32(feat, dirs, dir_group, params, dims: MlpDims, keep_act: bool):
    require_cuda(feat, params)
    feat = _f32c(feat)
    n = feat.shape[0]
    out = torch.empty((n, 4 if dirs is not None else 1), device=feat.device, dtype=torch.float32)
    act = torch.empty((mlp_act_rows(), n), device=feat.device, dtype=torch.float32) if keep_act else None
    check(lib().hbr_mlp_fwd_f32(ptr(feat), feat.stride(0), ptr(dirs), dir_group, n, ptr(params), C.byref(dims), ptr(out),
                                ptr(act), stream()))
    return out, act


def mlp_bwd_f32(feat, dirs, dir_group, params, dims: MlpDims, dout, act, want_dfeat, want_ddirs, dparams):
    n = feat.shape[0]
    dz = torch.empty_like(act)
    dfeat = torch.empty((n, dims.in0), device=feat.device, dtype=torch.float32) if want_dfeat else None
    ddirs = torch.zeros_like(dirs) if want_ddirs else None
    check(lib().hbr_mlp_bwd_f32(ptr(feat), feat.stride(0), ptr(dirs), dir_group, n, ptr(params), C.byref(dims), ptr(dout),
                                ptr(act), ptr(dz), ptr(dfeat), dims.in0, ptr(ddirs), ptr(dparams), stream()))
    return dfeat, ddirs


_tc_scratch = {}
_tc_image = {}


def mlp_tc_scratch(dims: MlpDims, device) -> torch.Tensor:
    key = (torch.device(device).index, dims.in0, dims.d_view)
    buf = _tc_scratch.get(key)
    if buf is None:
        buf = torch.empty(int(lib().hbr_mlp_tc_scratch_bytes(C.byref(dims))), device=device, dtype=torch.uint8)
        _tc_scratch[key] = buf
    return buf


def tc_operand(dtype=None) -> int:
    if dtype is None:
        dtype = torch.get_autocast_dtype("cuda") if torch.is_autocast_enabled() else torch.bfloat16
    if isinstance(dtype, int):
        if dtype in (HBR_F16, HBR_BF16):
            return dtype
        raise ValueError(f"operand format {dtype}")
    if dtype == torch.float16:
        return HBR_F16
    if dtype == torch.bfloat16:
        return HBR_BF16
    raise TypeError(f"the tensor-core MLP runs fp16 or bf16 operands, not {dtype}")


def _operand_torch_dtype(operand: int):
    return torch.float16 if operand == HBR_F16 else torch.bfloat16


def _feat_dtype(feat: torch.Tensor, operand: int) -> int:
    if feat.dtype == torch.float32:
        return HBR_F32
    if feat.dtype == _operand_torch_dtype(operand):
        return operand
    raise TypeError(f"features are {feat.dtype}; the MLP kernels take float32 or their own operand format")


# ... 186 lines not shown
```

### human_body_reconstruction_b200/vol_renderer.py

```python
from __future__ import annotations

import os
from collections import namedtuple
from typing import Optional, Tuple

import torch
import torch.nn as nn

from . import ops
from .encoder import PositionalEncoder
from .hash_encoding import HashEncoder
from .helper import calc_color, hierarchical_sampling, strat_sampler
from .test_hash import MLP_3D


class _FieldFn(torch.autograd.Function):

    @staticmethod
    def forward(ctx, pts, dirs, dir_group, enc, mlp, *params):
        geom, dims = enc._geom(), mlp._dims()
        dirs = dirs.float().contiguous()
        operand = ops.tc_operand()
        out, feat16 = ops.field_fwd_tc(pts, enc._flat_table(), geom, dirs, dir_group, mlp._flat_params(), dims, operand)
        ctx.enc, ctx.mlp, ctx.geom, ctx.dims, ctx.dir_group, ctx.operand = enc, mlp, geom, dims, dir_group, operand
        if enc._dp is not None:
            enc._dp.note_forward(enc)
            mlp._dp.note_forward(mlp)
        ctx.save_for_backward(pts, dirs, feat16, out)
        return out

    @staticmethod
    def backward(ctx, dout):
        pts, dirs, feat16, out = ctx.saved_tensors
        enc, mlp = ctx.enc, ctx.mlp
        L, T, F = enc.L, enc.T, enc.F
        flat = mlp._flat_params()
        dp = enc._dp
        if dp is not None:
            g, last_e = dp.enter_backward(enc)
            dflat, last_m = mlp._dp.enter_backward(mlp)
        else:
            g = torch.zeros((L, T, F), device=dout.device, dtype=torch.float32)
            dflat = torch.zeros_like(flat)
        ddirs = ops.field_bwd_tc(pts, ctx.geom, dirs, ctx.dir_group, flat, ctx.dims, feat16, out.detach(),
                                 dout.float().contiguous(), g, ctx.needs_input_grad[1], dflat, operand=ctx.operand,
                                 grad_scale=mlp.tc_grad_scale)
        if dp is not None:
            if last_m:
                mlp._dp.publish(mlp, dflat)
            if last_e:
                dp.publish(enc, g)
            return (None, ddirs, None, None, None) + (None,) * (L + len(mlp._ordered()))
        return (None, ddirs, None, None, None) + tuple(g[i] for i in range(L)) + tuple(mlp._grad_views(dflat))


class _FieldRaysFn(torch.autograd.Function):

    @staticmethod
    def forward(ctx, rays_o, rays_d, t, dirs, enc, mlp, *params):
        geom, dims = enc._geom(), mlp._dims()
        operand = ops.tc_operand()
        S = t.shape[-1]
        cur, side = torch.cuda.current_stream(), _side_stream(rays_o.device)
        flat = mlp._flat_params()
        side.wait_stream(cur)
        if FUSE_GATHER and rays_o.shape[0] * S <= FUSE_GATHER_MAX_POINTS and ops.field_scatter_supported(geom, dims):
            out, feat16 = ops.field_fwd_rays_tc(rays_o, rays_d, t, enc._flat_table(), geom, dirs, flat, dims, operand)
            with torch.cuda.stream(side):
                ops.mlp_tc_prepare(flat, dims, operand)
            cur.wait_stream(side)
        else:
            with torch.cuda.stream(side):
                ops.mlp_tc_prepare(flat, dims, operand)
            feat16 = ops.hash_encode_fwd_rays(rays_o, rays_d, t, enc._flat_table(), geom, operand)
            cur.wait_stream(side)
            out, _ = ops.mlp_fwd_tc(feat16, dirs, S, flat, dims, operand=operand, image_ready=True)
        ctx.enc, ctx.mlp, ctx.geom, ctx.dims, ctx.S, ctx.operand = enc, mlp, geom, dims, S, operand
        ctx.save_for_backward(rays_o, rays_d, t, dirs, feat16, out)
        ctx.want_tab = any(ctx.needs_input_grad[6:6 + enc.L])
        ctx.want_mlp = any(ctx.needs_input_grad[6 + enc.L:])
        ctx.g = None
        if ctx.want_tab:
            if enc._dp is not None:
                enc._dp.note_forward(enc)
            else:
                ctx.g = enc._zeroed_grad_async()
        if ctx.want_mlp and mlp._dp is not None:
            mlp._dp.note_forward(mlp)
        return out

    @staticmethod
    def backward(ctx, dout):
        rays_o, rays_d, t, dirs, feat16, out = ctx.saved_tensors
        enc, mlp = ctx.enc, ctx.mlp
        L, T, F = enc.L, enc.T, enc.F
        flat = mlp._flat_params()
        dpm = mlp._dp if ctx.want_mlp else None
        if dpm is not None:
            dflat, last_m = dpm.enter_backward(mlp)
        else:
            dflat, last_m = torch.zeros_like(flat), False
        if (FUSE_SCATTER and ctx.want_tab and ctx.want_mlp and enc._dp is None and dpm is None
                and feat16.shape[0] <= FUSE_SCATTER_MAX_POINTS and ops.field_scatter_supported(ctx.geom, ctx.dims)):
            if ctx.g is not None:
                g, ev = ctx.g
                ctx.g = None
                torch.cuda.current_stream().wait_event(ev)
            else:
                g = torch.zeros((L, T, F), device=dout.device, dtype=torch.float32)
            ddirs = ops.field_bwd_rays_tc(feat16, rays_o, rays_d, t, ctx.geom, dirs, flat, ctx.dims, out.detach(),
                                          dout.float().contiguous(), g, ctx.needs_input_grad[3], dflat, operand=ctx.operand,
                                          grad_scale=mlp.tc_grad_scale, defer_reduce=False)
            return (None, None, None, ddirs, None, None) + tuple(g[i] for i in range(L)) + tuple(mlp._grad_views(dflat))
        defer = ctx.want_tab
        n_pts = feat16.shape[0]
        dpe = enc._dp if ctx.want_tab else None
        plan, lm = None, False
        if dpe is not None:
            g, last = dpe.enter_backward(enc)
            plan = dpe.stream_plan(enc, L, n_pts) if last else None
            lm = plan is not None and STREAM_LEVEL_MAJOR and ops.mlp_level_major_ok(ctx.geom, ctx.dims, n_pts)
        dfeat, ddirs = ops.mlp_bwd_tc(feat16, dirs, ctx.S, flat, ctx.dims, out.detach(), dout.float().contiguous(), ctx.want_tab,
                                      ctx.needs_input_grad[3], dflat, operand=ctx.operand, grad_scale=mlp.tc_grad_scale,
                                      defer_reduce=defer, level_major=lm)
        cur, side = torch.cuda.current_stream(), _side_stream(dout.device)
        if defer:
            side.wait_stream(cur)
            with torch.cuda.stream(side):
                ops.mlp_tc_reduce_grads(ctx.dims, feat16.shape[0], dflat, dout.device)
            dflat.record_stream(side)

        def join_mlp():
            if defer:
                cur.wait_stream(side)
            if dpm is not None and last_m:
                dpm.publish(mlp, dflat)

        gm = (None,) * len(mlp._ordered()) if (dpm is not None or not ctx.want_mlp) else tuple(mlp._grad_views(dflat))
        if not ctx.want_tab:
            join_mlp()
            return (None, None, None, ddirs, None, None) + (None,) * L + gm
        if dpe is not None:
            if plan is not None:
                ev_pre = cur.record_event()
                if lm:
                    ops.hash_encode_bwd_rays_lm(rays_o, rays_d, t, dfeat, ctx.geom, g, plan, dpe.done)
                    need = ops.hash_bwd_lm_ctas(n_pts)
                else:
                    ops.hash_encode_bwd_rays_stream(rays_o, rays_d, t, dfeat, ctx.geom, g, plan, dpe.done)
                    need = ops.hash_bwd_stream_tiles(n_pts)
                with_mlp = dpm is dpe and last_m
                ev_mlp = side.record_event() if (defer and with_mlp) else None
                dpe.exchange_streamed(plan, need, after=(ev_pre, ev_mlp), include_mlp=with_mlp)
                if defer:
                    cur.wait_stream(side)
                if dpm is not None and last_m and not with_mlp:
                    dpm.publish(mlp, dflat)
                return (None, None, None, ddirs, None, None) + (None,) * L + gm
            for l0, l1 in (dpe.level_chunks(enc, L, feat16.shape[0]) if last else [(0, L)]):
                ops.hash_encode_bwd_rays(rays_o, rays_d, t, dfeat, ctx.geom, g, l0, l1)
                if l0 == 0:
                    join_mlp()
                if last:
                    dpe.publish(enc, g[l0:l1])
            return (None, None, None, ddirs, None, None) + (None,) * L + gm
        if ctx.g is not None:
            g, ev = ctx.g
            ctx.g = None
            torch.cuda.current_stream().wait_event(ev)
        else:
            g = torch.zeros((L, T, F), device=dout.device, dtype=torch.float32)
        ops.hash_encode_bwd_rays(rays_o, rays_d, t, dfeat, ctx.geom, g, 0, L)
        join_mlp()
        return (None, None, None, ddirs, None, None) + tuple(g[i] for i in range(L)) + gm


class _FieldCompactFn(torch.autograd.Function):

    @staticmethod
    def forward(ctx, rays_o, rays_d, t, dirs, grid, mu, sigma, enc, mlp, *params):
        geom, dims = enc._geom(), mlp._dims()
        operand = ops.tc_operand()
        pts_c, ray_c, rowmap, count = ops.compact_samples(rays_o, rays_d, t, grid, mu, sigma)
        cur, side = torch.cuda.current_stream(), _side_stream(rays_o.device)
# ... 453 lines not shown
```

### include/hbr.h

```cpp
#ifndef HBR_B200_H_
#define HBR_B200_H_

#include <stdint.h>

#ifdef __cplusplus
extern "C" {
#endif

#define HBR_ABI_VERSION 2
#define HBR_MAX_LEVELS 32

typedef enum {
  HBR_OK = 0,
  HBR_ERR_ARG = -1,
  HBR_ERR_CUDA = -2,
  HBR_ERR_UNSUPPORTED = -3
} hbr_status;

typedef enum { HBR_F32 = 0, HBR_F16 = 1, HBR_U8 = 2, HBR_BF16 = 3 } hbr_dtype;

typedef struct {
  float mu[3];
  float sigma;
  int32_t L;
  int32_t F;
  int32_t E;
  uint32_t T;
  float scale[HBR_MAX_LEVELS];
} hbr_hash_geom;

typedef struct {
  int32_t in0;
  int32_t d_view;
} hbr_mlp_dims;

int hbr_abi_version(void);
const char* hbr_last_error(void);
int64_t hbr_mlp_param_count(const hbr_mlp_dims* dims);
int64_t hbr_mlp_act_floats(void);

int hbr_hash_encode_fwd(const void* x, int x_dtype, int64_t n, const float* table,
                        const hbr_hash_geom* geom_host, float* y, int64_t y_stride, void* stream);

int hbr_hash_encode_bwd(const void* x, int x_dtype, int64_t n, const float* dy, int64_t dy_stride,
                        const hbr_hash_geom* geom_host, float* dtable, int level_begin, int level_end, void* stream);

int hbr_hash_encode_dx(const void* x, int x_dtype, int64_t n, const float* table, const hbr_hash_geom* geom_host,
                       const float* dy, int64_t dy_stride, float* dx, void* stream);

int hbr_hash_encode_fwd_rays(const float* rays_o, const float* rays_d, const float* t, int64_t t_ray_stride, int64_t R,
                             int64_t S, const float* table, const hbr_hash_geom* geom_host, void* y, int64_t y_stride,
                             int y_dtype, void* stream);
int hbr_hash_encode_bwd_rays(const float* rays_o, const float* rays_d, const float* t, int64_t t_ray_stride, int64_t R,
                             int64_t S, const float* dy, int64_t dy_stride, const hbr_hash_geom* geom_host, float* dtable,
                             int level_begin, int level_end, void* stream);

int64_t hbr_hash_bwd_stream_tiles(int64_t n);
int hbr_hash_encode_bwd_stream(const void* x, int x_dtype, int64_t n, const float* dy, int64_t dy_stride,
                               const hbr_hash_geom* geom_host, float* dtable, const int* level_bounds, int nchunks,
                               unsigned int* done, void* stream);
int hbr_hash_encode_bwd_rays_stream(const float* rays_o, const float* rays_d, const float* t, int64_t t_ray_stride, int64_t R,
                                    int64_t S, const float* dy, int64_t dy_stride, const hbr_hash_geom* geom_host,
                                    float* dtable, const int* level_bounds, int nchunks, unsigned int* done, void* stream);

int64_t hbr_hash_bwd_lm_ctas(int64_t n);
int hbr_hash_encode_bwd_lm(const void* x, int x_dtype, int64_t n, const float* dy_lm, const hbr_hash_geom* geom_host,
                           float* dtable, const int* level_bounds, int nchunks, unsigned int* done, void* stream);
int hbr_hash_encode_bwd_rays_lm(const float* rays_o, const float* rays_d, const float* t, int64_t t_ray_stride, int64_t R,
                                int64_t S, const float* dy_lm, const hbr_hash_geom* geom_host, float* dtable,
                                const int* level_bounds, int nchunks, unsigned int* done, void* stream);

int hbr_hash_indices(const void* x, int x_dtype, int64_t n, const hbr_hash_geom* geom_host,
                     int32_t* idx, float* w, void* stream);

int hbr_dir_encode(const void* d, int d_dtype, int64_t n, int dim, int num_freq, float* out, void* stream);

int hbr_mlp_fwd_f32(const float* feat, int64_t feat_stride, const float* dirs, int64_t dir_group, int64_t n,
                    const float* params, const hbr_mlp_dims* dims, float* out, float* act, void* stream);

int hbr_mlp_bwd_f32(const float* feat, int64_t feat_stride, const float* dirs, int64_t dir_group, int64_t n,
                    const float* params, const hbr_mlp_dims* dims, const float* dout, const float* act,
                    float* dz, float* dfeat, int64_t dfeat_stride, float* ddirs, float* dparams, void* stream);

int64_t hbr_mlp_tc_scratch_bytes(const hbr_mlp_dims* dims);
int hbr_mlp_tc_prepare(const float* params, const hbr_mlp_dims* dims, int operand, void* scratch, void* stream);
int hbr_mlp_tc_reduce_grads(const hbr_mlp_dims* dims, int64_t n, void* scratch, float* dparams, void* stream);
int hbr_mlp_fwd_tc(const void* feat, int feat_dtype, int64_t feat_stride, const float* dirs, int64_t dir_group, int64_t n,
                   const float* params, const hbr_mlp_dims* dims, int operand, float* out, void* scratch, int image_ready,
                   const unsigned long long* n_dev, const int32_t* dir_rows, void* stream);
#define HBR_DFEAT_LEVEL_MAJOR (-1)
int hbr_mlp_bwd_tc(const void* feat, int feat_dtype, int64_t feat_stride, const float* dirs, int64_t dir_group, int64_t n,
                   const float* params, const hbr_mlp_dims* dims, int operand, const float* out, const float* dout,
                   float* dfeat, int64_t dfeat_stride, float* ddirs, float* dparams, float grad_scale, void* scratch,
                   int image_ready, int defer_reduce, const unsigned long long* n_dev, const int32_t* dir_rows, void* stream);
int hbr_field_fwd_tc(const float* x, int64_t n, const float* table, const hbr_hash_geom* geom_host, const float* dirs,
                     int64_t dir_group, const float* params, const hbr_mlp_dims* dims, int operand, float* out,
                     void* feat16, void* scratch, void* stream);
int hbr_field_bwd_tc(const float* x, int64_t n, const hbr_hash_geom* geom_host, const float* dirs, int64_t dir_group,
                     const float* params, const hbr_mlp_dims* dims, int operand, const void* feat16, const float* out,
                     const float* dout, float* dtable, float* ddirs, float* dparams, float grad_scale, void* scratch,
                     void* stream);
int hbr_field_fwd_rays_tc(const float* rays_o, const float* rays_d, const float* t, int64_t t_ray_stride, int64_t R, int64_t S,
                          const float* table, const hbr_hash_geom* geom_host, const float* dirs, const float* params,
                          const hbr_mlp_dims* dims, int operand, float* out, void* feat16, void* scratch, int image_ready,
                          void* stream);
int hbr_field_bwd_rays_tc(const void* feat16, const float* rays_o, const float* rays_d, const float* t, int64_t t_ray_stride,
                          int64_t R, int64_t S, const hbr_hash_geom* geom_host, const float* dirs, const float* params,
                          const hbr_mlp_dims* dims, int operand, const float* out, const float* dout, float* dtable,
                          float* ddirs, float* dparams, float grad_scale, void* scratch, int image_ready, int defer_reduce,
                          void* stream);
int hbr_strat_depths(const float* lin, const float* u, float span, float count, int64_t S, float* t, void* stream);

int hbr_mse_pair_fwd(const float* a, const float* b, const float* gt, int64_t n, float scale, float* loss, void* stream);
int hbr_mse_pair_bwd(const float* a, const float* b, const float* gt, int64_t n, float scale, const float* gout, float* da,
                     float* db, void* stream);

int hbr_ray_points(const float* rays_o, const float* rays_d, const float* t, int64_t t_ray_stride,
                   int64_t R, int64_t S, float* pts, void* stream);

int hbr_occupancy_mask(const float* pts, int64_t n, const uint8_t* grid, int G, const float* mu3_host,
// ... 98 lines not shown
```

Baseline: 8.789 million.

## Launch kernels with programmatic dependent launch and trim small per-step overheads

Switches most kernel launches to cudaLaunchKernelEx with programmatic stream serialization and adds griddepcontrol wait/trigger at kernel entry. In the MLP kernels the wait is placed after mbarrier init and smem zeroing, so a kernel's prologue can overlap the tail of the previous one. It also makes the MSE forward a single 1024-thread CTA for small inputs, which removes the zero-init and the atomic. Other small cuts: the backward seed tensor is cached, and dflat zeroing moves to a side stream during forward. Calling launch_dependents at the very top lets dependent grids launch early and take SM resources, and the wait-before-read placement has to be correct in every kernel.

```diff
diff --git a/human_body_reconstruction_b200/_lib.py b/human_body_reconstruction_b200/_lib.py
--- a/human_body_reconstruction_b200/_lib.py
+++ b/human_body_reconstruction_b200/_lib.py
@@ -126,6 +126,7 @@
 SIGNATURES = {
     "hbr_abi_version": ([], C.c_int),
     "hbr_last_error": ([], C.c_char_p),
+    "hbr_set_pdl": ([_i32], C.c_int),
     "hbr_mlp_param_count": ([_dims_p], _i64),
     "hbr_mlp_act_floats": ([], _i64),
     "hbr_hash_encode_fwd": ([_vp, _i32, _i64, _vp, _geom_p, _vp, _i64, _vp], C.c_int),
diff --git a/human_body_reconstruction_b200/csrc/abi.cu b/human_body_reconstruction_b200/csrc/abi.cu
--- a/human_body_reconstruction_b200/csrc/abi.cu
+++ b/human_body_reconstruction_b200/csrc/abi.cu
@@ -1,5 +1,6 @@
 #include "common.cuh"
 #include <string.h>
+#include <atomic>
 
 namespace hbr {
 
@@ -29,7 +30,11 @@
   return cached;
 }
 
+static std::atomic<int> g_pdl{1};
+bool pdl_enabled() { return g_pdl.load(std::memory_order_relaxed) != 0; }
+
 }
 
 extern "C" int hbr_abi_version(void) { return HBR_ABI_VERSION; }
 extern "C" const char* hbr_last_error(void) { return hbr::err_buf(); }
+extern "C" int hbr_set_pdl(int on) { return hbr::g_pdl.exchange(on != 0 ? 1 : 0); }
diff --git a/human_body_reconstruction_b200/csrc/common.cuh b/human_body_reconstruction_b200/csrc/common.cuh
--- a/human_body_reconstruction_b200/csrc/common.cuh
+++ b/human_body_reconstruction_b200/csrc/common.cuh
@@ -31,6 +31,27 @@
 static inline int64_t ceil_div(int64_t a, int64_t b) { return (a + b - 1) / b; }
 static inline int64_t min64(int64_t a, int64_t b) { return a < b ? a : b; }
 int sm_count();
+
+bool pdl_enabled();
+
+__device__ __forceinline__ void pdl_wait() { asm volatile("griddepcontrol.wait;\n" ::: "memory"); }
+__device__ __forceinline__ void pdl_trigger() { asm volatile("griddepcontrol.launch_dependents;\n" ::: "memory"); }
+
+template <typename... KArgs, typename... Args>
+static inline cudaError_t launch_pdl(void (*kernel)(KArgs...), dim3 grid, dim3 block, size_t smem, cudaStream_t st,
+                                     Args&&... args) {
+  cudaLaunchAttribute attr[1];
+  attr[0].id = cudaLaunchAttributeProgrammaticStreamSerialization;
+  attr[0].val.programmaticStreamSerializationAllowed = 1;
+  cudaLaunchConfig_t cfg = {};
+  cfg.gridDim = grid;
+  cfg.blockDim = block;
+  cfg.dynamicSmemBytes = smem;
+  cfg.stream = st;
+  cfg.attrs = attr;
+  cfg.numAttrs = pdl_enabled() ? 1 : 0;
+  return cudaLaunchKernelEx(&cfg, kernel, static_cast<KArgs>(args)...);
+}
 
 constexpr uint32_t kPrimeY = 2654435761u;
 constexpr uint32_t kPrimeZ = 805459861u;
diff --git a/human_body_reconstruction_b200/csrc/composite.cu b/human_body_reconstruction_b200/csrc/composite.cu
--- a/human_body_reconstruction_b200/csrc/composite.cu
+++ b/human_body_reconstruction_b200/csrc/composite.cu
@@ -34,6 +34,8 @@
 
 template <typename XT>
 __global__ void dir_encode_kernel(const XT* __restrict__ d, long long n, int dim, int nf, float* __restrict__ out) {
+  pdl_wait();
+  pdl_trigger();
   const long long i = (long long)blockIdx.x * blockDim.x + threadIdx.x;
   const long long total = n * dim * nf;
   if (i >= total) return;
@@ -88,6 +90,8 @@
                      const uint8_t* __restrict__ mask, const int32_t* __restrict__ rowmap, long long R, int S,
                      float* __restrict__ C, float* __restrict__ w_out, float ert_tau, float* __restrict__ depth,
                      float* __restrict__ opac) {
+  pdl_wait();
+  pdl_trigger();
   const int lane = threadIdx.x & 31;
   const long long ray = (long long)blockIdx.x * kRaysPerCta + (threadIdx.x >> 5);
   if (ray >= R) return;
@@ -144,6 +148,8 @@
                      const uint8_t* __restrict__ mask, const int32_t* __restrict__ rowmap, long long R, int S,
                      const float* __restrict__ gC, float* __restrict__ drgb, long long drgb_st, float* __restrict__ dsig,
                      long long dsig_st, float ert_tau, const float* __restrict__ gD, const float* __restrict__ gA) {
+  pdl_wait();
+  pdl_trigger();
   const int lane = threadIdx.x & 31;
   const long long ray = (long long)blockIdx.x * kRaysPerCta + (threadIdx.x >> 5);
   if (ray >= R) return;
@@ -225,6 +231,8 @@
 hier_sample_kernel(float* __restrict__ w, const float* __restrict__ t, const float* __restrict__ u,
                    const float* __restrict__ cand, long long R, int S, int P2, int clamp_in_place,
                    float* __restrict__ t_fine) {
+  pdl_wait();
+  pdl_trigger();
   extern __shared__ float sm[];
   const int warp = threadIdx.x >> 5, lane = threadIdx.x & 31;
   float* cdf = sm + (size_t)warp * (S + P2);
@@ -313,9 +321,10 @@
   HBR_REQUIRE(d && out, "NULL pointer");
   const long long total = (long long)n * dim * num_freq;
   const unsigned grid = (unsigned)ceil_div(total, 256);
-  if (d_dtype == HBR_F16) dir_encode_kernel<__half><<<grid, 256, 0, as_stream(stream)>>>((const __half*)d, n, dim, num_freq, out);
-  else dir_encode_kernel<float><<<grid, 256, 0, as_stream(stream)>>>((const float*)d, n, dim, num_freq, out);
-  HBR_LAUNCH_CHECK();
+  if (d_dtype == HBR_F16)
+    HBR_CUDA(launch_pdl(dir_encode_kernel<__half>, grid, 256, 0, as_stream(stream), (const __half*)d, n, dim, num_freq, out));
+  else
+    HBR_CUDA(launch_pdl(dir_encode_kernel<float>, grid, 256, 0, as_stream(stream), (const float*)d, n, dim, num_freq, out));
   return HBR_OK;
 }
 
@@ -333,9 +342,8 @@
   if (int rc = check_composite(t, t_rs, rgb, sigma, R, S)) return rc;
   HBR_REQUIRE(C != nullptr, "C is NULL");
   if (!(ert_tau > 0.f)) ert_tau = 3.0e38f;
-  composite_fwd_kernel<false><<<(unsigned)ceil_div(R, kRaysPerCta), kRaysPerCta * 32, 0, as_stream(stream)>>>(
-      t, t_rs, rgb, rgb_st, sigma, sig_st, dn, dn_scalar, mask, rowmap, R, (int)S, C, w, ert_tau, nullptr, nullptr);
-  HBR_LAUNCH_CHECK();
+  HBR_CUDA(launch_pdl(composite_fwd_kernel<false>, (unsigned)ceil_div(R, kRaysPerCta), kRaysPerCta * 32, 0, as_stream(stream),
+                      t, t_rs, rgb, rgb_st, sigma, sig_st, dn, dn_scalar, mask, rowmap, R, (int)S, C, w, ert_tau, nullptr, nullptr));
   return HBR_OK;
 }
 
@@ -347,9 +355,8 @@
   if (int rc = check_composite(t, t_rs, rgb, sigma, R, S)) return rc;
   HBR_REQUIRE(C != nullptr, "C is NULL");
   if (!(ert_tau > 0.f)) ert_tau = 3.0e38f;
-  composite_fwd_kernel<true><<<(unsigned)ceil_div(R, kRaysPerCta), kRaysPerCta * 32, 0, as_stream(stream)>>>(
-      t, t_rs, rgb, rgb_st, sigma, sig_st, dn, dn_scalar, mask, rowmap, R, (int)S, C, w, ert_tau, depth, opacity);
-  HBR_LAUNCH_CHECK();
+  HBR_CUDA(launch_pdl(composite_fwd_kernel<true>, (unsigned)ceil_div(R, kRaysPerCta), kRaysPerCta * 32, 0, as_stream(stream),
+                      t, t_rs, rgb, rgb_st, sigma, sig_st, dn, dn_scalar, mask, rowmap, R, (int)S, C, w, ert_tau, depth, opacity));
   return HBR_OK;
 }
 
@@ -363,16 +370,14 @@
     HBR_REQUIRE((uintptr_t)drgb % 16 == 0, "packed gradient buffer must be 16-byte aligned");
   const unsigned grid = (unsigned)ceil_div(R, kRaysPerCta);
   cudaStream_t st = as_stream(stream);
-#define HBR_CB(N)                                                                                                      \
-  composite_bwd_kernel<N, MAPS><<<grid, kRaysPerCta * 32, 0, st>>>(t, t_rs, rgb, rgb_st, sigma, sig_st, dn, dn_scalar, \
-                                                                   mask, rowmap, R, (int)S, gC, drgb, drgb_st, dsig,   \
-                                                                   dsig_st, ert_tau, gD, gA)
-  if (S <= 128) HBR_CB(4);
-  else if (S <= 256) HBR_CB(8);
-  else if (S <= 512) HBR_CB(16);
-  else HBR_CB(32);
+#define HBR_CB(N)                                                                                                     \
+  launch_pdl(composite_bwd_kernel<N, MAPS>, grid, kRaysPerCta * 32, 0, st, t, t_rs, rgb, rgb_st, sigma, sig_st, dn, \
+             dn_scalar, mask, rowmap, R, (int)S, gC, drgb, drgb_st, dsig, dsig_st, ert_tau, gD, gA)
+  if (S <= 128) HBR_CUDA(HBR_CB(4));
+  else if (S <= 256) HBR_CUDA(HBR_CB(8));
+  else if (S <= 512) HBR_CUDA(HBR_CB(16));
+  else HBR_CUDA(HBR_CB(32));
 #undef HBR_CB
-  HBR_LAUNCH_CHECK();
   return HBR_OK;
 }
 
@@ -408,8 +413,7 @@
   while (P2 < 2 * S) P2 <<= 1;
   const size_t smem = (size_t)kHierWarps * (S + P2) * sizeof(float);
   HBR_CUDA(cudaFuncSetAttribute(hier_sample_kernel, cudaFuncAttributeMaxDynamicSharedMemorySize, (int)smem));
-  hier_sample_kernel<<<(unsigned)ceil_div(R, kHierWarps), kHierWarps * 32, smem, as_stream(stream)>>>(
-      w, t, u, cand, R, (int)S, P2, clamp_in_place, t_fine);
-  HBR_LAUNCH_CHECK();
-  return HBR_OK;
-}
+  HBR_CUDA(launch_pdl(hier_sample_kernel, (unsigned)ceil_div(R, kHierWarps), kHierWarps * 32, smem, as_stream(stream), w, t, u,
+                      cand, R, (int)S, P2, clamp_in_place, t_fine));
+  return HBR_OK;
+}
diff --git a/human_body_reconstruction_b200/csrc/hash_grid.cu b/human_body_reconstruction_b200/csrc/hash_grid.cu
--- a/human_body_reconstruction_b200/csrc/hash_grid.cu
+++ b/human_body_reconstruction_b200/csrc/hash_grid.cu
@@ -91,6 +91,8 @@
 hash_fwd_kernel(const typename PointSrc<XT>::type x, long long n, const float* __restrict__ table, YT* __restrict__ y,
                 long long y_stride, const __grid_constant__ HashGeom g, int y_fmt, const unsigned long long* __restrict__ n_dev) {
   extern __shared__ float tile[];
+  pdl_wait();
+  pdl_trigger();
   if (n_dev != nullptr) {
     n = min(n, (long long)__ldg(n_dev));
     if ((long long)blockIdx.x * kTilePts >= n) return;
@@ -541,8 +543,8 @@
   const size_t smem = (size_t)kTilePts * ((g.L * F) | 1) * sizeof(float);
   auto k = hash_fwd_kernel<F, POW2, RayPts, 0, 4, YT>;
   HBR_CUDA(cudaFuncSetAttribute(k, cudaFuncAttributeMaxDynamicSharedMemorySize, (int)smem));
-  k<<<(unsigned)ceil_div(n, kTilePts), kHashThreads, smem, st>>>(rs, n, table, static_cast<YT*>(y), ys, g, y_fmt, nullptr);
-  HBR_LAUNCH_CHECK();
+  HBR_CUDA(launch_pdl(k, (unsigned)ceil_div(n, kTilePts), kHashThreads, smem, st, rs, n, table, static_cast<YT*>(y), ys, g,
+                      y_fmt, nullptr));
   return HBR_OK;
 }
 template <int F, bool POW2>
@@ -562,8 +564,8 @@
   const size_t smem = (size_t)kTilePts * ((g.L * F) | 1) * sizeof(float);
   auto k = hash_fwd_kernel<F, POW2, float, 0, 4, YT>;
   HBR_CUDA(cudaFuncSetAttribute(k, cudaFuncAttributeMaxDynamicSharedMemorySize, (int)smem));
-  k<<<(unsigned)ceil_div(n, kTilePts), kHashThreads, smem, st>>>(x, n, table, static_cast<YT*>(y), ys, g, y_fmt, n_dev);
-  HBR_LAUNCH_CHECK();
+  HBR_CUDA(launch_pdl(k, (unsigned)ceil_div(n, kTilePts), kHashThreads, smem, st, x, n, table, static_cast<YT*>(y), ys, g,
+                      y_fmt, n_dev));
   return HBR_OK;
 }
 template <int F, bool POW2>
diff --git a/human_body_reconstruction_b200/csrc/mlp_tc_impl.cuh b/human_body_reconstruction_b200/csrc/mlp_tc_impl.cuh
--- a/human_body_reconstruction_b200/csrc/mlp_tc_impl.cuh
+++ b/human_body_reconstruction_b200/csrc/mlp_tc_impl.cuh
@@ -425,6 +425,8 @@
 __global__ void __launch_bounds__(256) mlp_prep_kernel(const float* __restrict__ params, int in0, int dv, uint8_t* img) {
   using SC = Scratch<K0P, KCP>;
   const MlpLayout m = make_layout(in0, dv);
+  pdl_wait();
+  pdl_trigger();
   if (blockIdx.x < kPrepCtas - 2) {
     constexpr int kChunks = WOfs<K0P, KCP>::total / 16;
     const int c = blockIdx.x * 256 + threadIdx.x;
@@ -450,6 +452,8 @@
 constexpr int kReduceSlices = 8;
 __global__ void __launch_bounds__(256) mlp_grad_reduce_kernel(const float* __restrict__ rows, int nrows, int row_floats,
                                                                int total, float* __restrict__ dparams) {
+  pdl_wait();
+  pdl_trigger();
   const int e = blockIdx.x * blockDim.x + threadIdx.x;
   if (e >= total) return;
   const int per = (nrows + kReduceSlices - 1) / kReduceSlices;
@@ -714,7 +718,6 @@
                   const uint8_t* __restrict__ image, long long* __restrict__ trace, const EncArgs enc,
                   const __grid_constant__ HashGeom geom, int feat16, const unsigned long long* __restrict__ n_dev,
                   const int32_t* __restrict__ dir_rows) {
-  const long long n = n_dev != nullptr ? min(n_arg, (long long)__ldg(n_dev)) : n_arg;
   using SM = FwdSmem<K0P, KCP, G>;
   using WO = WOfs<K0P, KCP>;
   constexpr int kGrpCols = 96;
@@ -741,6 +744,9 @@
       }
     fence_mbar_init();
   }
+  pdl_wait();
+  pdl_trigger();
+  const long long n = n_dev != nullptr ? min(n_arg, (long long)__ldg(n_dev)) : n_arg;
   if (GATH == 0) {
     if (image != nullptr) {
       copy_image_async(sm, image, SM::off_buf);
@@ -1096,7 +1102,6 @@
                   float* __restrict__ grad_rows, long long* __restrict__ trace, const EncArgs enc,
                   const __grid_constant__ HashGeom geom, float gscale, int feat16, const unsigned long long* __restrict__ n_dev,
                   const int32_t* __restrict__ dir_rows) {
-  const long long n = n_dev != nullptr ? min(n_arg, (long long)__ldg(n_dev)) : n_arg;
   const float ginv = 1.f / gscale;
   using SM = BwdSmem<K0P, KCP, G>;
   using WO = WOfs<K0P, KCP>;
@@ -1130,12 +1135,6 @@
     }
     fence_mbar_init();
   }
-  if (image != nullptr) {
-    copy_image_async(wsm, image, WO::total);
-    copy_image_async(sm + SM::off_bias, image + Scratch<K0P, KCP>::off_bias_f32, 6 * 64 * 4);
-  } else {
-    stage_weights_bf16<K0P, KCP>(params, m, wsm, nullptr, nullptr, bias);
-  }
   {
     for (int e = threadIdx.x; e < G * SM::grp_bytes / 16; e += blockDim.x)
       reinterpret_cast<uint4*>(sm + SM::off_grp)[e] = make_uint4(0, 0, 0, 0);
@@ -1152,6 +1151,15 @@
         reinterpret_cast<uint4*>(gb + SM::c1 + 8 * kCg)[e] = ones4;
       }
     }
+  }
+  pdl_wait();
+  pdl_trigger();
+  const long long n = n_dev != nullptr ? min(n_arg, (long long)__ldg(n_dev)) : n_arg;
+  if (image != nullptr) {
+    copy_image_async(wsm, image, WO::total);
+    copy_image_async(sm + SM::off_bias, image + Scratch<K0P, KCP>::off_bias_f32, 6 * 64 * 4);
+  } else {
+    stage_weights_bf16<K0P, KCP>(params, m, wsm, nullptr, nullptr, bias);
   }
   cp_async_wait_all();
   fence_async_smem();
@@ -1648,12 +1656,12 @@
                          cudaStream_t st) {
   constexpr int smem = FwdSmem<K0P, KCP, G>::total;
   const int grid = (int)min64(ceil_div(ceil_div(n, kTile), G), sm_count());
-  if (scratch != nullptr && !image_ready) mlp_prep_kernel<K0P, KCP><<<kPrepCtas, 256, 0, st>>>(params, in0, dv, scratch);
+  if (scratch != nullptr && !image_ready)
+    HBR_CUDA(launch_pdl(mlp_prep_kernel<K0P, KCP>, kPrepCtas, 256, 0, st, params, in0, dv, scratch));
   auto kern = mlp_fwd_tc_kernel<K0P, KCP, G, false, ENC>;
   HBR_CUDA(cudaFuncSetAttribute(kern, cudaFuncAttributeMaxDynamicSharedMemorySize, smem));
-  kern<<<grid, G * kTile, smem, st>>>(feat, feat_stride, dirs, dir_group, n, params, in0, dv, out, scratch, nullptr, enc,
-                                             geom, feat16, n_dev, dir_rows);
-  HBR_LAUNCH_CHECK();
+  HBR_CUDA(launch_pdl(kern, grid, G * kTile, smem, st, feat, feat_stride, dirs, dir_group, n, params, in0, dv, out, scratch,
+                      nullptr, enc, geom, feat16, n_dev, dir_rows));
   return HBR_OK;
 }
 
@@ -1665,9 +1673,8 @@
   const int grid = (int)min64(ceil_div(ceil_div(n, kTile), G), sm_count());
   auto kern = mlp_fwd_tc_kernel<32, 48, G, false, false, GATH>;
   HBR_CUDA(cudaFuncSetAttribute(kern, cudaFuncAttributeMaxDynamicSharedMemorySize, smem));
-  kern<<<grid, G * kTile + GATH * 32, smem, st>>>(nullptr, 32, dirs, dir_group, n, params, 32, dv, out, image, nullptr, enc, geom,
-                                                  1, nullptr, nullptr);
-  HBR_LAUNCH_CHECK();
+  HBR_CUDA(launch_pdl(kern, grid, G * kTile + GATH * 32, smem, st, nullptr, 32, dirs, dir_group, n, params, 32, dv, out, image,
+                      nullptr, enc, geom, 1, nullptr, nullptr));
   return HBR_OK;
 }
 
@@ -1681,7 +1688,8 @@
   constexpr int smem = BwdSmem<K0P, KCP, G>::total;
   const int grid = (int)min64(ceil_div(ceil_div(n, kTile), G), sm_count());
   const bool rows = scratch != nullptr && dparams != nullptr && grid <= SC::kMaxRows;
-  if (scratch != nullptr && !image_ready) mlp_prep_kernel<K0P, KCP><<<kPrepCtas, 256, 0, st>>>(params, in0, dv, scratch);
+  if (scratch != nullptr && !image_ready)
+    HBR_CUDA(launch_pdl(mlp_prep_kernel<K0P, KCP>, kPrepCtas, 256, 0, st, params, in0, dv, scratch));
   auto kern = mlp_bwd_tc_kernel<K0P, KCP, G, false, ENC, SCAT>;
   HBR_CUDA(cudaFuncSetAttribute(kern, cudaFuncAttributeMaxDynamicSharedMemorySize, smem));
   if constexpr (SCAT > 0) {
@@ -1696,15 +1704,15 @@
     HBR_REQUIRE(regs >= kScatRegs && regs <= kGroupRegs && 4 * regs <= 512 && G * kGroupRegs + (4 - G) * kScatRegs <= 4 * regs,
                 "fused backward kernel compiled with %d registers per thread: the setmaxnreg budget does not hold", regs);
   }
-  kern<<<grid, G * kTile + SCAT * 32 + 32, smem, st>>>(feat, feat_stride, dirs, dir_group, n, params, in0, dv, out, dout, dfeat,
-                                           dfeat_stride, ddirs, dparams, scratch,
-                                           rows ? reinterpret_cast<float*>(scratch + SC::off_grad) : nullptr, nullptr, enc, geom, gscale, feat16, n_dev, dir_rows);
+  HBR_CUDA(launch_pdl(kern, grid, G * kTile + SCAT * 32 + 32, smem, st, feat, feat_stride, dirs, dir_group, n, params, in0, dv,
+                      out, dout, dfeat, dfeat_stride, ddirs, dparams, scratch,
+                      rows ? reinterpret_cast<float*>(scratch + SC::off_grad) : nullptr, nullptr, enc, geom, gscale, feat16, n_dev,
+                      dir_rows));
   if (rows && !defer_reduce) {
     const int total = make_layout(in0, dv).total;
-    mlp_grad_reduce_kernel<<<dim3((total + 255) / 256, kReduceSlices), 256, 0, st>>>(
-        reinterpret_cast<const float*>(scratch + SC::off_grad), grid, SC::kRowFloats, total, dparams);
-  }
-  HBR_LAUNCH_CHECK();
+    HBR_CUDA(launch_pdl(mlp_grad_reduce_kernel, dim3((total + 255) / 256, kReduceSlices), 256, 0, st,
+                        reinterpret_cast<const float*>(scratch + SC::off_grad), grid, SC::kRowFloats, total, dparams));
+  }
   return HBR_OK;
 }
 
@@ -1714,15 +1722,13 @@
   const int grid = (int)min64(ceil_div(ceil_div(n, kTile), G), sm_count());
   HBR_REQUIRE(grid <= SC::kMaxRows, "grid %d exceeds the gradient rows", grid);
   const int total = make_layout(in0, dv).total;
-  mlp_grad_reduce_kernel<<<dim3((total + 255) / 256, kReduceSlices), 256, 0, st>>>(
-      reinterpret_cast<const float*>(scratch + SC::off_grad), grid, SC::kRowFloats, total, dparams);
-  HBR_LAUNCH_CHECK();
+  HBR_CUDA(launch_pdl(mlp_grad_reduce_kernel, dim3((total + 255) / 256, kReduceSlices), 256, 0, st,
+                      reinterpret_cast<const float*>(scratch + SC::off_grad), grid, SC::kRowFloats, total, dparams));
   return HBR_OK;
 }
 template <int K0P, int KCP>
 static int prepare_tc(const float* params, int in0, int dv, uint8_t* scratch, cudaStream_t st) {
-  mlp_prep_kernel<K0P, KCP><<<kPrepCtas, 256, 0, st>>>(params, in0, dv, scratch);
-  HBR_LAUNCH_CHECK();
+  HBR_CUDA(launch_pdl(mlp_prep_kernel<K0P, KCP>, kPrepCtas, 256, 0, st, params, in0, dv, scratch));
   return HBR_OK;
 }
 
diff --git a/human_body_reconstruction_b200/csrc/occupancy.cu b/human_body_reconstruction_b200/csrc/occupancy.cu
--- a/human_body_reconstruction_b200/csrc/occupancy.cu
+++ b/human_body_reconstruction_b200/csrc/occupancy.cu
@@ -45,6 +45,8 @@
                        long long R, int S, const uint8_t* __restrict__ grid, int G, Mu3o mu, float sigma,
                        float* __restrict__ pts_c, int32_t* __restrict__ ray_c, int32_t* __restrict__ rowmap,
                        unsigned long long* __restrict__ count) {
+  pdl_wait();
+  pdl_trigger();
   const int lane = threadIdx.x & 31;
   const long long ray = (long long)blockIdx.x * kCompactWarps + (threadIdx.x >> 5);
   if (ray >= R) return;
@@ -123,8 +125,7 @@
   if (R == 0) return HBR_OK;
   HBR_REQUIRE(rays_o && rays_d && t && grid && G > 0 && mu3 && pts_c && ray_c && rowmap && count, "NULL pointer");
   Mu3o mu{{mu3[0], mu3[1], mu3[2]}};
-  compact_samples_kernel<<<(unsigned)ceil_div(R, kCompactWarps), kCompactWarps * 32, 0, as_stream(stream)>>>(
-      rays_o, rays_d, t, t_ray_stride, R, (int)S, grid, G, mu, sigma, pts_c, ray_c, rowmap, count);
-  HBR_LAUNCH_CHECK();
+  HBR_CUDA(launch_pdl(compact_samples_kernel, (unsigned)ceil_div(R, kCompactWarps), kCompactWarps * 32, 0, as_stream(stream),
+                      rays_o, rays_d, t, t_ray_stride, R, (int)S, grid, G, mu, sigma, pts_c, ray_c, rowmap, count));
   return HBR_OK;
 }
diff --git a/human_body_reconstruction_b200/csrc/step_glue.cu b/human_body_reconstruction_b200/csrc/step_glue.cu
--- a/human_body_reconstruction_b200/csrc/step_glue.cu
+++ b/human_body_reconstruction_b200/csrc/step_glue.cu
@@ -4,13 +4,18 @@
 
 __global__ void strat_depths_kernel(const float* __restrict__ lin, const float* __restrict__ u, float span, float count,
                                     long long S, float* __restrict__ t) {
+  pdl_wait();
+  pdl_trigger();
   const long long i = (long long)blockIdx.x * blockDim.x + threadIdx.x;
   if (i < S) t[i] = __fadd_rn(__ldg(lin + i), __fdiv_rn(__fmul_rn(__ldg(u + i), span), count));
 }
 
-__global__ void __launch_bounds__(256)
+constexpr long long kMseOneCta = 1 << 15;
+__global__ void __launch_bounds__(1024)
 mse_pair_fwd_kernel(const float* __restrict__ a, const float* __restrict__ b, const float* __restrict__ gt, long long n,
                     double inv_n, float* __restrict__ loss) {
+  pdl_wait();
+  pdl_trigger();
   float facc = 0.f;
   for (long long i = (long long)blockIdx.x * blockDim.x + threadIdx.x; i < n; i += (long long)gridDim.x * blockDim.x) {
     const float g = __ldg(gt + i);
@@ -24,19 +29,22 @@
   double acc = (double)facc;
 #pragma unroll
   for (int o = 16; o > 0; o >>= 1) acc += __shfl_xor_sync(kFull, acc, o);
-  __shared__ double part[8];
+  __shared__ double part[32];
   const int warp = threadIdx.x >> 5, lane = threadIdx.x & 31;
   if (lane == 0) part[warp] = acc;
   __syncthreads();
   if (threadIdx.x == 0) {
     double s = 0.0;
-    for (int w = 0; w < 8; ++w) s += part[w];
-    atomicAdd(loss, (float)(s * inv_n));
+    for (int w = 0; w < (int)(blockDim.x >> 5); ++w) s += part[w];
+    if (gridDim.x == 1) *loss = (float)(s * inv_n);
+    else atomicAdd(loss, (float)(s * inv_n));
   }
 }
 __global__ void mse_pair_bwd_kernel(const float* __restrict__ a, const float* __restrict__ b, const float* __restrict__ gt,
                                     long long n, float two_over_n, const float* __restrict__ gout, float* __restrict__ da,
                                     float* __restrict__ db) {
+  pdl_wait();
+  pdl_trigger();
   const long long i = (long long)blockIdx.x * blockDim.x + threadIdx.x;
   if (i >= n) return;
   const float s = __ldg(gout) * two_over_n, g = __ldg(gt + i);
@@ -52,24 +60,27 @@
   HBR_REQUIRE(S >= 0 && count != 0.f, "S=%lld count=%g", (long long)S, (double)count);
   if (S == 0) return HBR_OK;
   HBR_REQUIRE(lin && u && t, "NULL pointer");
-  strat_depths_kernel<<<(unsigned)ceil_div(S, 256), 256, 0, as_stream(stream)>>>(lin, u, span, count, S, t);
-  HBR_LAUNCH_CHECK();
+  HBR_CUDA(launch_pdl(strat_depths_kernel, (unsigned)ceil_div(S, 256), 256, 0, as_stream(stream), lin, u, span, count, S, t));
   return HBR_OK;
 }
 
 extern "C" int hbr_mse_pair_fwd(const float* a, const float* b, const float* gt, int64_t n, float scale, float* loss,
                                 void* stream) {
   HBR_REQUIRE(n >= 1 && a && gt && loss, "bad argument");
+  if (n <= kMseOneCta) {
+    HBR_CUDA(launch_pdl(mse_pair_fwd_kernel, 1, 1024, 0, as_stream(stream), a, b, gt, n, (double)scale / (double)n, loss));
+    return HBR_OK;
+  }
   const int grid = (int)min64(ceil_div(n, 256 * 4), (long long)sm_count() * 4);
-  mse_pair_fwd_kernel<<<grid, 256, 0, as_stream(stream)>>>(a, b, gt, n, (double)scale / (double)n, loss);
-  HBR_LAUNCH_CHECK();
+  HBR_CUDA(cudaMemsetAsync(loss, 0, sizeof(float), as_stream(stream)));
+  HBR_CUDA(launch_pdl(mse_pair_fwd_kernel, grid, 256, 0, as_stream(stream), a, b, gt, n, (double)scale / (double)n, loss));
   return HBR_OK;
 }
 
 extern "C" int hbr_mse_pair_bwd(const float* a, const float* b, const float* gt, int64_t n, float scale, const float* gout,
                                 float* da, float* db, void* stream) {
   HBR_REQUIRE(n >= 1 && a && gt && gout && da && (b == nullptr || db != nullptr), "bad argument");
-  mse_pair_bwd_kernel<<<(unsigned)ceil_div(n, 256), 256, 0, as_stream(stream)>>>(a, b, gt, n, 2.f * scale / (float)n, gout, da, db);
-  HBR_LAUNCH_CHECK();
+  HBR_CUDA(launch_pdl(mse_pair_bwd_kernel, (unsigned)ceil_div(n, 256), 256, 0, as_stream(stream), a, b, gt, n,
+                      2.f * scale / (float)n, gout, da, db));
   return HBR_OK;
 }
diff --git a/human_body_reconstruction_b200/graph.py b/human_body_reconstruction_b200/graph.py
--- a/human_body_reconstruction_b200/graph.py
+++ b/human_body_reconstruction_b200/graph.py
@@ -40,6 +40,7 @@
         self.loss: Optional[torch.Tensor] = None
         self.graph: Optional[torch.cuda.CUDAGraph] = None
         self._warmup = warmup
+        self._seeds = {}
 
     def _step(self):
         rays_o, rays_d, dir_norm, gt = self.rays_o, self.rays_d, self.dir_norm, self.gt
@@ -49,10 +50,17 @@
             Cr, Cf, _ = self.renderer.vol_render(self.model, rays_d, rays_o, num_samples=self.num_samples,
                                                  update_mask=False, dir_norm=dir_norm, hierarchical=self.hierarchical)
             loss = self.loss_fn(Cr, Cf, gt)
-        loss.backward()
+        loss.backward(self._seed(loss))
         for o in self.optimizers:
             o.step()
         return loss
+
+    def _seed(self, loss):
+        key = (loss.shape, loss.dtype, loss.device)
+        seed = self._seeds.get(key)
+        if seed is None:
+            seed = self._seeds[key] = torch.ones_like(loss, memory_format=torch.contiguous_format)
+        return seed
 
     @staticmethod
     def pack_batch(rays_o, rays_d, dir_norm, gt, pin: bool = False) -> torch.Tensor:
diff --git a/human_body_reconstruction_b200/ops.py b/human_body_reconstruction_b200/ops.py
--- a/human_body_reconstruction_b200/ops.py
+++ b/human_body_reconstruction_b200/ops.py
@@ -547,7 +547,7 @@
         b = _f32c(b) if b is not None else None
         if a.shape != gt.shape or (b is not None and b.shape != gt.shape):
             raise ValueError("MsePair: shapes differ")
-        loss = torch.zeros((), device=a.device, dtype=torch.float32)
+        loss = torch.empty((), device=a.device, dtype=torch.float32)
         check(lib().hbr_mse_pair_fwd(ptr(a), ptr(b), ptr(gt), a.numel(), float(scale), ptr(loss), stream()))
         ctx.save_for_backward(a, b, gt)
         ctx.scale = float(scale)
diff --git a/human_body_reconstruction_b200/vol_renderer.py b/human_body_reconstruction_b200/vol_renderer.py
--- a/human_body_reconstruction_b200/vol_renderer.py
+++ b/human_body_reconstruction_b200/vol_renderer.py
@@ -64,6 +64,12 @@
         cur, side = torch.cuda.current_stream(), _side_stream(rays_o.device)
         flat = mlp._flat_params()
         side.wait_stream(cur)
+        ctx.dflat = None
+        if any(ctx.needs_input_grad[6 + enc.L:]) and mlp._dp is None:
+            with torch.cuda.stream(side):
+                dflat = torch.zeros_like(flat)
+                ctx.dflat = (dflat, side.record_event())
+            dflat.record_stream(cur)
         if FUSE_GATHER and rays_o.shape[0] * S <= FUSE_GATHER_MAX_POINTS and ops.field_scatter_supported(geom, dims):
             out, feat16 = ops.field_fwd_rays_tc(rays_o, rays_d, t, enc._flat_table(), geom, dirs, flat, dims, operand)
             with torch.cuda.stream(side):
@@ -98,8 +104,12 @@
         dpm = mlp._dp if ctx.want_mlp else None
         if dpm is not None:
             dflat, last_m = dpm.enter_backward(mlp)
+        elif ctx.dflat is not None:
+            (dflat, ev), last_m = ctx.dflat, False
+            torch.cuda.current_stream().wait_event(ev)
         else:
             dflat, last_m = torch.zeros_like(flat), False
+        ctx.dflat = None
         if (FUSE_SCATTER and ctx.want_tab and ctx.want_mlp and enc._dp is None and dpm is None
                 and feat16.shape[0] <= FUSE_SCATTER_MAX_POINTS and ops.field_scatter_supported(ctx.geom, ctx.dims)):
             if ctx.g is not None:
diff --git a/include/hbr.h b/include/hbr.h
--- a/include/hbr.h
+++ b/include/hbr.h
@@ -36,6 +36,7 @@
 
 int hbr_abi_version(void);
 const char* hbr_last_error(void);
+int hbr_set_pdl(int on);
 int64_t hbr_mlp_param_count(const hbr_mlp_dims* dims);
 int64_t hbr_mlp_act_floats(void);
 
```

Result: faster. 9.053 million (median of 6 runs) (+3.0%).
